# cl-volume-renderer/cl-volume-renderer

Hardware: AMD Instinct MI355X
Metric: msamples_per_sec (higher is better)
Workload: dtype f32

## Files before the change

### cl_volume_renderer_amd/csrc/bounce_device.hpp

```cpp
#pragma once
#include "render_device.hpp"

namespace clvr {

__device__ __forceinline__ VolumePacked make_volume(const RenderArgs &a) {
  return VolumePacked{a.grec, a.stepb, a.volume_lin, a.sdf_lin, a.X, a.Y, a.Z, a.NBX, a.NBY};
}

__device__ __forceinline__ uint32_t udivmod24(uint32_t n, uint32_t d, uint32_t &rem) {
  uint32_t q = (uint32_t)((float)n * __builtin_amdgcn_rcpf((float)d));
  uint32_t qd;
  asm("v_mul_u32_u24 %0, %1, %2" : "=v"(qd) : "v"(q), "v"(d));
  int32_t r = (int32_t)(n - qd);
  if (r < 0) { q -= 1u; r += (int32_t)d; }
  if (r >= (int32_t)d) { q += 1u; r -= (int32_t)d; }
  rem = (uint32_t)r;
  return q;
}

__device__ __forceinline__ unsigned prefix_count(unsigned long long mask) {
  return __builtin_amdgcn_mbcnt_hi((unsigned)(mask >> 32), __builtin_amdgcn_mbcnt_lo((unsigned)mask, 0u));
}
__device__ __forceinline__ unsigned lane_id() { return prefix_count(~0ull); }

enum : int { ST_IDLE = 0, ST_MARCH = 1, ST_CERT = 2, ST_EVENT = 8 };
enum : int { EV_START = 3,
             EV_HIT_COLOR_PENDING = 4,
             EV_CHECK = 5 };
constexpr int kCertNever = 255;

template <int MODE>
__device__ __forceinline__ void finish_item(const RenderArgs &a, int64_t entry, uint32_t hit, uint32_t gx, uint32_t gy,
                                            uint32_t bv_r, uint32_t bv_g, uint32_t bv_b) {
  const uint32_t cr = (bv_r / 2u) & 0xFFFFu, cg = (bv_g / 2u) & 0xFFFFu, cb = (bv_b / 2u) & 0xFFFFu;
  if (MODE == CLWH_ACCUM_VOXEL_CACHE && a.grants == nullptr) {
    cache_add(a.cache, entry, cr, cg, cb, 0u);
  } else {
    const unsigned long long packed = (unsigned long long)cr | ((unsigned long long)cg << 16) |
                                      ((unsigned long long)cb << 32) | (1ull << 48);
    atomicAdd(a.delta + hit, packed);
  }
  if (a.contrib_out) {
    uint32_t *q = a.contrib_out + ((size_t)gy * (size_t)a.launch_w + gx) * 4;
    q[0] = cr; q[1] = cg; q[2] = cb; q[3] = 1u;
  }
}

constexpr int kFixupDwords = 32;

__device__ __forceinline__ bool certify_exit(const RenderArgs &a, f3 p, f3 d, int budget, int &away) {
  const unsigned cx = min((unsigned)(int)p.x >> a.macro_shift, (unsigned)a.MNX - 1u), cy = min((unsigned)(int)p.y >> a.macro_shift, (unsigned)a.MNY - 1u),
                 cz = min((unsigned)(int)p.z >> a.macro_shift, (unsigned)a.MNZ - 1u);
  const unsigned octant = (d.x < 0.0f ? 1u : 0u) | (d.y < 0.0f ? 2u : 0u) | (d.z < 0.0f ? 4u : 0u);
  const int entry = a.macro[(((cz * (unsigned)a.MNY + cy) * (unsigned)a.MNX + cx) << 3) | octant];
  const bool refused = (entry & (int)kCertRefused) != 0;
  const int box_min = refused ? 0 : entry;
  away = refused ? ((entry & 0x7F) - 1) << a.macro_shift : 0;
  const float dmin = fminf(fminf(fabsf(d.x), fabsf(d.y)), fabsf(d.z));
  const float dsum = d.x + d.y + d.z;
  const float T = (float)((budget - 5) * box_min);
  const float fx = d.x < 0.0f ? p.x : (float)a.X - p.x, fy = d.y < 0.0f ? p.y : (float)a.Y - p.y, fz = d.z < 0.0f ? p.z : (float)a.Z - p.z;
  const bool leaves = T * fabsf(d.x) >= fx || T * fabsf(d.y) >= fy || T * fabsf(d.z) >= fz;
  return box_min != 0 && budget > 5 && leaves && dmin >= 0.0009765625f && dsum == dsum;
}
__device__ __forceinline__ bool start_certificate(uint32_t mask, f3 d, float dmin_needed) {
  const unsigned octant = (d.x < 0.0f ? 1u : 0u) | (d.y < 0.0f ? 2u : 0u) | (d.z < 0.0f ? 4u : 0u);
  const float dmin = fminf(fminf(fabsf(d.x), fabsf(d.y)), fabsf(d.z));
  const float dsum = d.x + d.y + d.z;
  return ((mask >> octant) & 1u) != 0u && dmin >= dmin_needed && dsum == dsum;
}
__device__ __forceinline__ f3 hull_direction(unsigned k) {
  static_assert(kHullGrid == 64, "cell centres are odd multiples of 1/64");
  const float u = (float)(2 * (int)(k & 63u) - 63) * 0.015625f, v = (float)(2 * (int)((k >> 6) & 63u) - 63) * 0.015625f;
  const float z = (1.0f - fabsf(u)) - fabsf(v);
  const float x = z >= 0.0f ? u : copysignf(1.0f - fabsf(v), u), y = z >= 0.0f ? v : copysignf(1.0f - fabsf(u), v);
  const float r = __builtin_amdgcn_rsqf((x * x + y * y) + z * z);
  return f3{x * r, y * r, z * r};
}
__device__ __forceinline__ bool certify_exit(const RenderArgs &a, f3 p, f3 d, int budget) {
  int away;
  return certify_exit(a, p, d, budget, away);
}

template <int SMALL>
__device__ __forceinline__ void index_tables_to_lds(VolumePacked &vol, const RenderArgs &a, int threads) {
  extern __shared__ uint32_t lds_parts[];
  if (SMALL == 2) {
    vol.parts = lds_parts;
    vol.parts_y0 = a.X;
    vol.parts_z0 = a.X + a.Y;
    for (int k = (int)threadIdx.x; k < a.X + a.Y + a.Z; k += threads)
      lds_parts[k] = k < a.X ? vol.part_x<1>((unsigned)k) : (k < a.X + a.Y ? vol.part_y<1>((unsigned)(k - a.X)) : vol.part_z<1>((unsigned)(k - a.X - a.Y)));
  }
}
__device__ __forceinline__ unsigned home_queue_of(const RenderArgs &a, unsigned waves_per_block) {
  unsigned home_queue = (unsigned)__builtin_amdgcn_s_getreg((3 << 11) | 20) & 7u;
  if (a.unit_affinity == 1) home_queue = (blockIdx.x * waves_per_block + (threadIdx.x >> 6)) & 7u;
  if (a.unit_affinity == 2) home_queue = 0u;
  return home_queue;
}

#ifdef CLVR_BOUNCE_STATS
constexpr bool kBounceStats = true;
constexpr bool kStartCertVerify = (CLVR_BOUNCE_STATS + 0) != 2;
#else
constexpr bool kBounceStats = false;
constexpr bool kStartCertVerify = false;
#endif
template <bool ON> struct BounceStatsT;
template <> struct BounceStatsT<false> {
  __device__ void step(int) {}
  __device__ void cert_begin(int, int) {}
  __device__ void cert_end(int, int) {}
  __device__ void closing_half(int) {}
  __device__ void event_phase(int) {}
  __device__ void refill(uint32_t) {}
  __device__ void fresh_items(int, int) {}
  __device__ void swap_point() {}
  __device__ void start_cert(bool, bool) {}
  __device__ void hull_cert(bool, bool, bool) {}
  __device__ void hull_more(bool, bool, bool, bool) {}
  __device__ void hull_fired(bool, bool) {}
  __device__ void march_end(uint32_t *, int) {}
  template <bool TWO_RAYS> __device__ void flush(uint32_t *) {}
};
template <> struct BounceStatsT<true> {
  uint32_t step_iters = 0, step_lanes = 0, event_phases = 0, event_lanes = 0, refills = 0, refill_lanes = 0;
  uint32_t ev_kind[4] = {0, 0, 0, 0};
  uint32_t cert_phases = 0, cert_lanes = 0, cert_granted = 0;
  uint32_t step_idle = 0;
  uint32_t swaps = 0;
  uint32_t closing = 0, marching_before = 0;
  __device__ __forceinline__ void step(int st) {
    step_iters += 1; step_lanes += (uint32_t)__popcll(__ballot(st == ST_MARCH));
    step_idle += (uint32_t)__popcll(__ballot(st == ST_IDLE));
  }
  __device__ __forceinline__ void cert_begin(int st, int n_cert) {
    cert_phases += 1; cert_lanes += (uint32_t)n_cert;
    marching_before = (uint32_t)__popcll(__ballot(st == ST_MARCH));
  }
  __device__ __forceinline__ void cert_end(int st, int n_cert) { cert_granted += (uint32_t)(n_cert - (__popcll(__ballot(st == ST_MARCH)) - (int)marching_before)); }
  __device__ __forceinline__ void closing_half(int st) {
    closing = (uint32_t)__popcll(__ballot(st >= ST_EVENT));
    event_lanes += closing;
    ev_kind[1] += (uint32_t)__popcll(__ballot(st == ST_EVENT + EV_EXIT || st == ST_EVENT + EV_CHECK));
    ev_kind[2] += (uint32_t)__popcll(__ballot(st == ST_EVENT + EV_HIT || st == ST_EVENT + EV_HIT_COLOR_PENDING));
    ev_kind[3] += (uint32_t)__popcll(__ballot(st == ST_EVENT + EV_NONE));
  }
  __device__ __forceinline__ void event_phase(int st) {
    if (__ballot(st >= ST_EVENT) != 0ull) { event_phases += 1; event_lanes += (uint32_t)__popcll(__ballot(st >= ST_EVENT)); }
  }
  __device__ __forceinline__ void refill(uint32_t count) { refills += 1; refill_lanes += count; }
  __device__ __forceinline__ void fresh_items(int st, int o) {
    const uint32_t n_fresh = (uint32_t)__popcll(__ballot(st == ST_EVENT + EV_START && o == 1));
    ev_kind[0] += n_fresh; event_lanes += n_fresh;
    if (closing + n_fresh != 0u) event_phases += 1;
  }
  __device__ __forceinline__ void swap_point() { swaps += 1; }
  uint32_t start_tried = 0, start_granted = 0;
  bool start_open = false;
  __device__ __forceinline__ void start_cert(bool tried, bool granted) {
    start_tried += (uint32_t)__popcll(__ballot(tried)); start_granted += (uint32_t)__popcll(__ballot(granted));
    start_open = start_open || granted;
  }
  uint32_t hull_tried = 0, hull_granted = 0, hull_both = 0;
  bool hull_open = false;
  __device__ __forceinline__ void hull_cert(bool tried, bool granted, bool both) {
    hull_tried += (uint32_t)__popcll(__ballot(tried)); hull_granted += (uint32_t)__popcll(__ballot(granted));
    hull_both += (uint32_t)__popcll(__ballot(both));
    hull_open = hull_open || granted;
  }
  uint32_t more_tried[3] = {0, 0, 0}, more_granted[3] = {0, 0, 0};
  int more_open = -1;
  __device__ __forceinline__ void hull_more(bool rebound_tried, bool rebound_granted, bool armed, bool first_leg) {
    more_tried[0] += (uint32_t)__popcll(__ballot(armed && first_leg)); more_tried[2] += (uint32_t)__popcll(__ballot(armed && !first_leg));
    more_tried[1] += (uint32_t)__popcll(__ballot(rebound_tried)); more_granted[1] += (uint32_t)__popcll(__ballot(rebound_granted));
    if (rebound_granted) more_open = 1;
  }
  __device__ __forceinline__ void hull_fired(bool fired, bool first_leg) {
    more_granted[0] += (uint32_t)__popcll(__ballot(fired && first_leg)); more_granted[2] += (uint32_t)__popcll(__ballot(fired && !first_leg));
    if (fired) more_open = first_leg ? 0 : 2;
  }
  __device__ __forceinline__ void march_end(uint32_t *counters, int ev) {
    if (start_open && ev != EV_EXIT) atomicAdd(&counters[CTR_START_WRONG], 1u);
    if (hull_open && ev != EV_EXIT) atomicAdd(&counters[CTR_HULL_WRONG], 1u);
    if (more_open >= 0 && ev != EV_EXIT) atomicAdd(&counters[CTR_HULL_DEFER + 3 * more_open + 2], 1u);
    start_open = false;
    hull_open = false;
    more_open = -1;
  }
  template <bool TWO_RAYS> __device__ __forceinline__ void flush(uint32_t *counters) {
    atomicAdd(&counters[CTR_STEP_ITERS], step_iters); atomicAdd(&counters[CTR_STEP_LANES], step_lanes);
    atomicAdd(&counters[CTR_EVENT_PHASES], event_phases); atomicAdd(&counters[CTR_EVENT_LANES], event_lanes);
    atomicAdd(&counters[CTR_REFILLS], refills); atomicAdd(&counters[CTR_REFILL_LANES], refill_lanes);
    if (TWO_RAYS) { atomicAdd(&counters[CTR_SWAPS], swaps); return; }
    for (int k = 0; k < 4; ++k) atomicAdd(&counters[CTR_EV_KIND + k], ev_kind[k]);
    atomicAdd(&counters[CTR_CERT_PHASES], cert_phases); atomicAdd(&counters[CTR_CERT_LANES], cert_lanes);
    atomicAdd(&counters[CTR_CERT_GRANTED], cert_granted); atomicAdd(&counters[CTR_STEP_IDLE], step_idle);
    atomicAdd(&counters[CTR_START_TRIED], start_tried); atomicAdd(&counters[CTR_START_GRANTED], start_granted);
    atomicAdd(&counters[CTR_HULL_TRIED], hull_tried); atomicAdd(&counters[CTR_HULL_GRANTED], hull_granted); atomicAdd(&counters[CTR_HULL_BOTH], hull_both);
    for (int k = 0; k < 3; ++k) { atomicAdd(&counters[CTR_HULL_DEFER + 3 * k], more_tried[k]); atomicAdd(&counters[CTR_HULL_DEFER + 3 * k + 1], more_granted[k]); }
  }
};
using BounceStats = BounceStatsT<kBounceStats>;

}
```

### cl_volume_renderer_amd/csrc/clwh_context.hip

```cpp
#include <algorithm>
#include <cstdio>
#include <cstdlib>
#include <cstring>
#include <mutex>
#include <new>

#include "clwh_host.hpp"

using namespace clvr;

static thread_local int g_last_hip_error = 0;
void clvr::note_hip_error(hipError_t e) { g_last_hip_error = (int)e; }

static std::atomic<uint64_t> g_content_version{0};
static std::mutex g_cells_mutex;
static std::map<const void *, std::weak_ptr<VersionCell>> g_version_cells;
void clwh_touch(clwh_mem *m) { m->cell->v.store(++g_content_version, std::memory_order_relaxed); }

static std::shared_ptr<VersionCell> version_cell_of(const void *dptr) {
  std::lock_guard<std::mutex> lock(g_cells_mutex);
  auto it = g_version_cells.find(dptr);
  if (it != g_version_cells.end())
    if (auto live = it->second.lock()) return live;
  auto cell = std::make_shared<VersionCell>();
// ... 50 lines not shown
    return rc;
  }
  ctx->classes.cache[source] = j;
  out = j;
  return CLWH_OK;
}

int clvr::ensure_classes(clwh_ctx *ctx, const std::shared_ptr<JitTf> &jit, const clwh_mem *volume, TfDev &tf_out, const uint8_t **cls_out) {
  TfClasses &c = ctx->classes;
  if (c.cls.ptr && c.vol == volume->dptr && c.vol_ver == volume->version() && c.source == jit->source) {
    tf_out = c.tf;
    *cls_out = c.cls.as<uint8_t>();
    return CLWH_OK;
  }
  if (!jit->module) {
    HIP_TRY(hipModuleLoadData(&jit->module, jit->code.data()));
    HIP_TRY(hipModuleGetFunction(&jit->classify, jit->module, "clvr_tf_classify"));
  }
  const size_t voxels = volume->dims[0] * volume->dims[1] * volume->dims[2];
  CLWH_TRY(c.cls.reserve(ctx->stream, voxels));
  constexpr int kColors = CLWH_TF_MAX_RULES;
  CLWH_TRY(c.palette.reserve(ctx->stream, (kColors + 2) * sizeof(unsigned long long)));
  unsigned long long *palette = c.palette.as<unsigned long long>();
  HIP_TRY(hipMemsetAsync(palette, 0xFF, kColors * sizeof(unsigned long long), ctx->stream));
  HIP_TRY(hipMemsetAsync(palette + kColors, 0, 2 * sizeof(unsigned long long), ctx->stream));
  const void *vol = volume->dptr;
  int X = (int)volume->dims[0], Y = (int)volume->dims[1], Z = (int)volume->dims[2], max_colors = kColors;
  unsigned char *cls = c.cls.as<unsigned char>();
  int *error = reinterpret_cast<int *>(palette + kColors);
  int *border = reinterpret_cast<int *>(palette + kColors + 1);
  void *args[] = {&vol, &X, &Y, &Z, &cls, &palette, &max_colors, &error, &border};
  const size_t blocks = std::min<size_t>((voxels + 255u) / 256u, (size_t)1u << 23);
  HIP_TRY(hipModuleLaunchKernel(jit->classify, (unsigned)blocks, 1, 1, 256, 1, 1, 0, ctx->stream, args, nullptr));
  unsigned long long host[kColors + 2];
  HIP_TRY(hipMemcpyAsync(host, palette, sizeof host, hipMemcpyDeviceToHost, ctx->stream));
  HIP_TRY(hipStreamSynchronize(ctx->stream));
  c.vol = nullptr;
  if ((int)(host[kColors] & 0xFFFFFFFFull) != 0) return CLWH_ERR_TF_UNSUPPORTED;
  TfDev t;
  std::memset(&t, 0, sizeof t);
  t.opaque = 1;
  for (int k = 0; k < kColors && host[k] != ~0ull; ++k) {
    t.rules[k].flags = (host[k] >> 32) & 1ull ? TF_WRITES_COLOR : 0u;
    t.rules[k].color = (uint32_t)(host[k] & 0xFFFFFFFFull);
    t.n = k + 1;
  }
  t.border_class = (int32_t)(host[kColors + 1] & 0xFFull);
  c.tf = t;
  c.vol = volume->dptr;
  c.vol_ver = volume->version();
  c.source = jit->source;
  tf_out = t;
  *cls_out = cls;
  return CLWH_OK;
}


Tuning clvr::tuning_from_environment() {
  Tuning t;
  auto clamped = [](const char *e, int lo, int hi) { return std::max(lo, std::min(hi, std::atoi(e))); };
  if (const char *e = std::getenv("CLWH_TUNE_STEP")) t.step_min_lanes = clamped(e, 0, 64);
  if (const char *e = std::getenv("CLWH_TUNE_REFILL")) t.refill_min_lanes = clamped(e, 0, 64);
  if (const char *e = std::getenv("CLWH_TUNE_LITERAL_GRADIENT")) t.literal_gradient = std::atoi(e) != 0;
  if (const char *e = std::getenv("CLWH_TUNE_AFFINITY")) t.unit_affinity = std::atoi(e);
  if (const char *e = std::getenv("CLWH_TUNE_QUEUES")) t.unit_queues = clamped(e, 1, 8);
  if (const char *e = std::getenv("CLWH_TUNE_GROUP")) t.unit_group = std::max(1, std::atoi(e));
  if (const char *e = std::getenv("CLWH_TUNE_CHUNK_BLOCK_LOG2")) t.unit_block_log2 = clamped(e, 0, 8);
  if (const char *e = std::getenv("CLWH_TUNE_BLOCKS")) t.bounce_max_blocks = (uint32_t)std::max(1, std::atoi(e));
  if (const char *e = std::getenv("CLWH_TUNE_MACRO_SHIFT")) t.macro_shift = std::atoi(e);
  if (const char *e = std::getenv("CLWH_TUNE_LONG_LAUNCH")) t.force_long_launch = std::atoi(e) != 0;
  if (const char *e = std::getenv("CLWH_TUNE_BOUNCE_RAYS")) t.bounce_rays = std::atoi(e) == 2 ? 2 : 1;
  if (const char *e = std::getenv("CLWH_TUNE_SDF")) t.sdf_front = std::strcmp(e, "front") == 0;
  if (const char *e = std::getenv("CLWH_TUNE_DIST_LINES")) t.dist_lines = std::strcmp(e, "scan") == 0 ? 1 : std::strcmp(e, "search") == 0 ? 2 : 0;
  if (const char *e = std::getenv("CLWH_TUNE_LABEL_STATS")) t.label_stats = std::strcmp(e, "item") == 0 ? 1 : std::strcmp(e, "direct") == 0 ? 2 : 0;
  if (const char *e = std::getenv("CLWH_TUNE_SLICE_COARSE")) t.slice_coarse = std::atoi(e) != 0;
  if (const char *e = std::getenv("CLWH_TUNE_SDFBIT_WAVES")) t.sdfbit_waves = std::atoi(e) == 16 ? 16 : 8;
  if (const char *e = std::getenv("CLWH_TUNE_SDFBIT_GRID")) t.sdfbit_grid = std::max(1, std::atoi(e));
  if (const char *e = std::getenv("CLWH_TUNE_SDFBIT_REC")) t.sdfbit_rec_lds = std::strcmp(e, "lds") == 0 ? 1 : 0;
  if (const char *e = std::getenv("CLWH_TUNE_CERT")) t.cert_min_step = clamped(e, 0, 127);
  if (const char *e = std::getenv("CLWH_TUNE_CERT_HINT")) t.cert_hint = std::atoi(e) != 0;
  if (const char *e = std::getenv("CLWH_TUNE_START_CERT")) t.start_cert = std::atoi(e) != 0;
  if (const char *e = std::getenv("CLWH_TUNE_HULL_CERT")) t.hull_cert = std::atoi(e) != 0;
  if (const char *e = std::getenv("CLWH_TUNE_HULL_DEFER")) t.hull_defer = std::atoi(e) != 0;
  return t;
}

int clvr::check_device_flags(clwh_ctx *ctx) {
  PassScratch &p = ctx->pass;
  if (!p.fixup_overflow_pending || !p.sticky_flags.ptr) return CLWH_OK;
  uint32_t flag = 0;
  HIP_TRY(hipMemcpyAsync(&flag, p.sticky_flags.ptr, sizeof flag, hipMemcpyDeviceToHost, ctx->stream));
  HIP_TRY(hipStreamSynchronize(ctx->stream));
  p.fixup_overflow_pending = false;
  if (!flag) return CLWH_OK;
  HIP_TRY(hipMemsetAsync(p.sticky_flags.ptr, 0, sizeof(uint32_t), ctx->stream));
  return CLWH_ERR_INTERNAL_OVERFLOW;
}

int clvr::timed_begin(clwh_ctx *ctx, int which, hipEvent_t *end) {
  LaunchTimers &t = ctx->timers;
  if (!t.enabled) return CLWH_OK;
  if (t.used == t.pairs.size()) {
    LaunchTimers::Pair &fresh = t.pairs.emplace_back();
    int rc = fresh.begin.ensure(hipEventDefault);
    if (rc == CLWH_OK) rc = fresh.end.ensure(hipEventDefault);
    if (rc != CLWH_OK) {
      t.pairs.pop_back();
      return rc;
    }
  }
  LaunchTimers::Pair &p = t.pairs[t.used++];
  p.which = which;
  HIP_TRY(hipEventRecord(p.begin.ev, ctx->stream));
  *end = p.end.ev;
  return CLWH_OK;
}

static int order_streams(clwh_ctx *ctx, hipStream_t first, hipStream_t then) {
  HIP_TRY(hipSetDevice(ctx->device));
  CLWH_TRY(ctx->handoff.ensure(hipEventDisableTiming));
  HIP_TRY(hipEventRecord(ctx->handoff.ev, first));
  HIP_TRY(hipStreamWaitEvent(then, ctx->handoff.ev, 0));
  return CLWH_OK;
}

extern "C" {

int clwh_ctx_create_on_stream(int device, void *hip_stream, clwh_ctx **out) {
  if (!out) return CLWH_ERR_INVALID_VALUE;
  *out = nullptr;
  int count = 0;
  hipError_t e = hipGetDeviceCount(&count);
  if (e != hipSuccess || count <= 0) {
    note_hip_error(e);
    return CLWH_ERR_NO_DEVICE;
  }
  if (device < 0 || device >= count) return CLWH_ERR_NO_DEVICE;
  HIP_TRY(hipSetDevice(device));
  clwh_ctx *c = new (std::nothrow) clwh_ctx();
  if (!c) return CLWH_ERR_OUT_OF_MEMORY;
  c->device = device;
  c->stream = (hipStream_t)hip_stream;
  c->own_stream = false;
  c->tune = tuning_from_environment();
  *out = c;
  return CLWH_OK;
}

int clwh_ctx_create(int device, clwh_ctx **out) {
  CLWH_TRY(clwh_ctx_create_on_stream(device, nullptr, out));
  hipStream_t s;
  hipError_t e = hipStreamCreateWithFlags(&s, hipStreamNonBlocking);
  if (e != hipSuccess) {
    note_hip_error(e);
    delete *out;
    *out = nullptr;
    return CLWH_ERR_HIP;
  }
  (*out)->stream = s;
  (*out)->own_stream = true;
  return CLWH_OK;
}

int clwh_ctx_destroy(clwh_ctx *ctx) {
  if (!ctx) return CLWH_ERR_INVALID_VALUE;
  (void)hipSetDevice(ctx->device);
// ... 225 lines not shown
```

### cl_volume_renderer_amd/csrc/clwh_host.hpp

```cpp
#pragma once

#include <atomic>
#include <deque>
#include <map>
#include <memory>
#include <string>
#include <vector>

#include "clwh_internal.hpp"

namespace clvr {

void note_hip_error(hipError_t e);
inline int hip_failed(hipError_t e) {
  note_hip_error(e);
  return e == hipErrorOutOfMemory ? CLWH_ERR_OUT_OF_MEMORY : CLWH_ERR_HIP;
}
#define HIP_TRY(expr)                                   \
  do {                                                  \
    hipError_t _e = (expr);                             \
    if (_e != hipSuccess) return clvr::hip_failed(_e);  \
  } while (0)
#define CLWH_TRY(expr)                \
  do {                                \
// ... 14 lines not shown
  template <class T>
  T *as() const { return static_cast<T *>(ptr); }
  void *release() {
    void *p = ptr;
    ptr = nullptr;
    bytes = 0;
    return p;
  }
  int reserve(hipStream_t stream, size_t need, bool *reallocated = nullptr) {
    if (reallocated) *reallocated = bytes < need;
    if (bytes >= need) return CLWH_OK;
    if (ptr) {
      HIP_TRY(hipStreamSynchronize(stream));
      HIP_TRY(hipFree(ptr));
      (void)release();
    }
    HIP_TRY(hipMalloc(&ptr, need));
    bytes = need;
    return CLWH_OK;
  }
};

struct Event : NoCopy {
  hipEvent_t ev = nullptr;
  ~Event() { if (ev) (void)hipEventDestroy(ev); }
  int ensure(unsigned flags) {
    if (!ev) HIP_TRY(hipEventCreateWithFlags(&ev, flags));
    return CLWH_OK;
  }
};

struct PinnedWord : NoCopy {
  uint32_t *ptr = nullptr;
  ~PinnedWord() { if (ptr) (void)hipHostFree(ptr); }
  int ensure() {
    if (!ptr) HIP_TRY(hipHostMalloc((void **)&ptr, 64, hipHostMallocDefault));
    return CLWH_OK;
  }
};

int tf_jit_compile(const char *user_source, std::vector<char> &code, std::string &log);
struct JitTf {
  std::string source;
  std::vector<char> code;
  hipModule_t module = nullptr;
  hipFunction_t classify = nullptr;
};

struct PackedScene {
  int device = 0;
  DeviceBuffer data;
  const void *vol = nullptr, *sdf = nullptr;
  uint64_t vol_ver = 0, sdf_ver = 0;
  TfDev tf{};
  std::string tf_identity;
  int32_t macro_shift = 0;
  bool start_table = false;
  bool hull_table = false;
  int32_t dims[3] = {0, 0, 0};
  uint64_t generation = 0;
  Event ready;
  bool stale = false;
  ~PackedScene();
};

struct VersionCell {
  std::atomic<uint64_t> v{0};
};


struct Tuning {
  int32_t step_min_lanes = 0;
  int32_t refill_min_lanes = 0;
  int32_t macro_shift = 0;
  int32_t bounce_rays = 1;
  int32_t force_long_launch = 0;
  int32_t literal_gradient = 0;
  int32_t unit_block_log2 = 4;
  int32_t unit_group = 1, unit_affinity = 0, unit_queues = 8;
  int32_t cert_hint = 1;
  int32_t start_cert = 1;
  int32_t hull_cert = 1;
  int32_t hull_defer = 1;
  int32_t cert_min_step = -1;
  uint32_t bounce_max_blocks = 2048;
  int32_t sdfbit_waves = 8;
  int32_t sdfbit_grid = 512;
  int32_t sdfbit_rec_lds = 0;
  int32_t sdf_front = 0;
  int32_t dist_lines = 0;
  int32_t label_stats = 0;
  int32_t slice_coarse = 1;
};
Tuning tuning_from_environment();

struct PrimaryHits {
  struct Key {
    float cam_pos[3], cam_dir[3];
    int32_t frame_w, frame_h, launch_w, launch_h, tile_rank, tile_world;
    int64_t cache_entries;
    int32_t mode, shading;
    uint64_t packed_generation;
    const void *env;
    uint64_t env_version;
    int32_t env_w, env_h;
  } key{};
  bool valid = false;
  DeviceBuffer pix_slot, hits;
  DeviceBuffer hull_codes;
  DeviceBuffer hull_planes;
  uint32_t n_hits = 0;
  bool n_hits_known = false;
  PinnedWord host_n_hits;
  Event n_hits_event;
  bool n_hits_in_flight = false;
  uint32_t last_known_n_hits = 0;
};

struct PassScratch {
  static constexpr size_t kCounters = CTR_QUEUE_STRIDE * 10;
  DeviceBuffer counters;
  DeviceBuffer fixups, delta;
  DeviceBuffer sticky_flags;
  bool fixup_overflow_pending = false;
};

struct VoxelPlan {
  DeviceBuffer plan;
  DeviceBuffer temp;
  bool valid = false;
  uint32_t n = 0;
};

struct TfClasses {
  std::map<std::string, std::shared_ptr<JitTf>> cache;
  DeviceBuffer cls;
  DeviceBuffer palette;
  const void *vol = nullptr;
  uint64_t vol_ver = 0;
  std::string source;
  TfDev tf{};
};

struct SdfScratch {
  DeviceBuffer counters;
  DeviceBuffer flags;
  DeviceBuffer bits;
#ifdef CLVR_SDFBIT_TIMING
  DeviceBuffer timing;
#endif
};

struct TileScratch {
  DeviceBuffer tiles, seeds;
  PinnedWord host;
};

struct GrowScratch {
  DeviceBuffer admissible;
  TileScratch work;
};

struct LabelScratch {
  DeviceBuffer admissible, keys, temp, counters;
  PinnedWord host;
};
// ... 211 lines not shown
```

### cl_volume_renderer_amd/csrc/clwh_internal.hpp

```cpp
#pragma once

#include <hip/hip_runtime.h>
#include <stdint.h>

#include "../../include/clwh.h"

namespace clvr {

struct TfRuleDev {
  int32_t v_lo, v_hi, g_lo, g_hi;
  uint32_t flags;
  uint32_t color;
};
struct TfDev {
  int32_t n;
  int32_t uses_gradient;
  int32_t literal_gradient_taps;
  int32_t opaque;
  int32_t border_class;
  TfRuleDev rules[CLWH_TF_MAX_RULES];
};

enum : uint32_t { TF_USE_GRADIENT = 1u, TF_WRITES_COLOR = 2u, TF_TERMINAL = 4u };

struct HitRec {
  float origin[3];
  float direction[3];
  float normal[3];
  uint32_t color;
  int32_t entry_lo;
  int32_t entry_hi;
  uint32_t xy;
  uint32_t pslot;
  uint32_t start_free;
  uint32_t pad;
};
static_assert(sizeof(HitRec) == 64, "HitRec must be one 64-byte line");

enum : uint32_t { PIX_HIT = 0x80000000u };

constexpr uint32_t kCertMinStep = 2u;
constexpr uint32_t kCertRefused = 0x80u;

enum : uint32_t {
  CTR_HITS = 0, CTR_FIXUPS = 2,
  CTR_STEP_ITERS = 8, CTR_STEP_LANES, CTR_EVENT_PHASES, CTR_EVENT_LANES, CTR_REFILLS, CTR_REFILL_LANES,
  CTR_EV_KIND,
  CTR_CERT_PHASES = CTR_EV_KIND + 4, CTR_CERT_LANES, CTR_CERT_GRANTED,
  CTR_SWAPS, CTR_STEP_IDLE,
  CTR_START_TRIED, CTR_START_GRANTED, CTR_START_WRONG,
  CTR_HULL_TRIED, CTR_HULL_GRANTED, CTR_HULL_BOTH, CTR_HULL_WRONG,
  CTR_STATS_END,
  CTR_QUEUE_STRIDE = 32,
  CTR_HULL_DEFER = CTR_QUEUE_STRIDE * 9, CTR_HULL_DEFER_END = CTR_HULL_DEFER + 9,
};
struct RenderArgs {
  int32_t X, Y, Z;
  const uint2 *grec;
  const uint8_t *stepb;
  const int16_t *volume_lin;
  const int8_t *sdf_lin;
  const uint8_t *macro;
  int32_t MNX, MNY, MNZ, macro_shift;
  int32_t cert_min_step;
  int32_t cert_min_lanes;
  int32_t cert_hint;
  const uint8_t *start_free;
  float start_cert_dmin;
  const float4 *hull;
  uint32_t *hull_codes;
  float hull_delta0;
  uint32_t *hull_planes;
  float hull_defer_delta0;
  int32_t NBX, NBY;
  const uint32_t *env;
  int32_t env_w, env_h;
  uint32_t *cache;
  int64_t cache_entries;
  uint32_t *frame;
  int32_t frame_w, frame_h;
  int32_t launch_w, launch_h;
  int32_t tiles_x, tiles_y, tiles_per_row;
  int32_t tile_rank, tile_world;
  float cam_pos[3];
  float cam_dir[3];
  int32_t mode;
  float4 *accum;
  unsigned long long *delta;
  const uint32_t *grants;
  uint32_t *pix_slot;
  HitRec *hits;
  uint32_t *counters;
  uint32_t *fixups;
  uint32_t fixup_capacity;
  uint32_t *sticky_flags;
  uint32_t n_hits;
  uint32_t n_hits_estimate;
  int32_t n_hits_on_device;
  int32_t shading;
  int64_t *hit_index_out;
  uint32_t *contrib_out;
  uint32_t num_tile_slots;
  int32_t n_seeds;
  int32_t seeds[CLWH_MAX_SEEDS];
  int32_t step_min_lanes;
  int32_t refill_min_lanes;
  int32_t force_long_launch;
  int32_t bounce_rays;
  uint32_t bounce_max_blocks;
  int32_t unit_group;
  int32_t unit_block_log2;
  int32_t unit_queues;
  int32_t unit_affinity;
  TfDev tf;
};

struct RepackArgs {
  const int16_t *volume;
  const int8_t *sdf;
  int32_t X, Y, Z;
  int32_t NBX, NBY, NBZ;
  uint2 *grec;
  uint8_t *stepb;
  uint32_t *brick_min;
  const uint8_t *cls_in;
  TfDev tf;
};

struct SdfArgs {
  const int16_t *volume;
  int32_t X, Y, Z;
  int8_t *ping;
  int8_t *pong;
  int32_t max_iterations;
  int32_t iteration;
  int32_t *counters;
  int32_t *done;
  int32_t *counter_out;
  const uint8_t *cls_in;
  TfDev tf;
};

hipError_t launch_repack(const RepackArgs &a, hipStream_t s);
inline int macro_cell_shift(int X, int Y, int Z, int forced) {
  if (forced >= 3 && forced <= 8) return forced;
  auto cells = [&](int sh) { return (int64_t)((X >> sh) + 1) * ((Y >> sh) + 1) * ((Z >> sh) + 1); };
  int shift = 4;
  if (cells(4) > 40000) {
    shift = 5;
    while (shift < 8 && cells(shift) > 300000) ++shift;
  }
  return shift;
}
hipError_t launch_macro_table(const uint32_t *brick_min, int NBX, int NBY, int NBZ, uint8_t *macro, int X, int Y, int Z, int shift, hipStream_t s);
hipError_t launch_start_table(const uint8_t *stepb, uint8_t *table, uint32_t *regular, int2 *ends, int X, int Y, int Z, int NBX, int NBY, int NBZ, hipStream_t s);
inline int start_cert_cap(int X, int Y, int Z) {
  const int longest = X > Y ? (X > Z ? X : Z) : (Y > Z ? Y : Z);
  return longest / 2 < 127 ? longest / 2 : 127;
}
inline float start_cert_dmin(int X, int Y, int Z) {
  const double longest = (double)(X > Y ? (X > Z ? X : Z) : (Y > Z ? Y : Z));
  const double reach = 1.7320508075688772 * (longest + 1.0), cap = (double)start_cert_cap(X, Y, Z);
  for (int k = 1; k <= 64; ++k) {
    const double dmin = (double)k / 64.0;
    double t = 0.0;
    for (int step = 0; step < 70 - 5 && t <= reach; ++step) {
      const double m = (double)(long long)(t * dmin) - 2.0;
      const double bound = m > cap ? cap : m;
      t += bound < 1.0 ? 1.0 : bound;
    }
    if (t > reach) return (float)dmin;
  }
  return 2.0f;
}
constexpr int kHullGrid = 64;
constexpr int kHullPlanes = kHullGrid * kHullGrid;
constexpr float kHullSlack = 0.0625f;
constexpr int kHullMaxDim = 2048;
inline float hull_cert_delta0(int X, int Y, int Z) {
  const double longest = (double)(X > Y ? (X > Z ? X : Z) : (Y > Z ? Y : Z));
  const double reach = 1.7320508075688772 * (longest + 1.0), cap = (double)start_cert_cap(X, Y, Z);
  for (int k = 1; k <= 64; ++k) {
    const double delta0 = (double)k / 64.0;
    double t = 0.0;
    for (int step = 0; step < 70 - 5 && t <= reach; ++step) {
      const double m = (double)(long long)(t * delta0 / 1.7320508075688772) - 2.0;
      const double bound = m > cap ? cap : m;
      t += bound < 1.0 ? 1.0 : bound;
    }
    if (t > reach) return (float)delta0;
  }
  return 2.0f;
}
constexpr int kHullDeferSteps = 3;
constexpr float kHullDeferDeficit = 1.5f;
constexpr int kHullMarginScale = 16;
inline float hull_defer_delta0(int X, int Y, int Z) {
  const double longest = (double)(X > Y ? (X > Z ? X : Z) : (Y > Z ? Y : Z));
  const double reach = 1.7320508075688772 * (longest + 1.0), cap = (double)start_cert_cap(X, Y, Z);
  for (int k = 1; k <= 64; ++k) {
    const double delta0 = (double)k / 64.0;
    double t = 0.0;
    for (int step = 0; step < 70 - 5 - kHullDeferSteps && t <= reach; ++step) {
      const double m = (double)(long long)(t * delta0 / 1.7320508075688772) - 2.0;
      const double bound = m > cap ? cap : m;
      t += bound < 1.0 ? 1.0 : bound;
    }
    if (t > reach) return (float)delta0;
  }
  return 2.0f;
}
hipError_t launch_hull_table(const int2 *ends, const uint32_t *regular, float4 *hull, int X, int Y, int Z, hipStream_t s);
constexpr uint64_t kStartTableBudget = 2ull << 30;
hipError_t launch_primary(const RenderArgs &a, hipStream_t s);
hipError_t launch_bounce(const RenderArgs &a, hipStream_t s);
inline bool bounce_queues_fit(uint32_t n_hits, int32_t unit_block_log2, int32_t n_seeds) {
  return (uint64_t)(((n_hits + 63u) >> 6) + 8u * (1u << unit_block_log2)) * (uint64_t)n_seeds < (1ull << 24);
}
hipError_t launch_env_fixup(const RenderArgs &a, hipStream_t s);
hipError_t launch_commit(const RenderArgs &a, hipStream_t s);
constexpr int64_t kVoxKeyInvalid = (int64_t)1 << 38;
constexpr int64_t kVoxKeyNone = ((int64_t)1 << 38) + 1;
hipError_t launch_vox_keys(const RenderArgs &a, int64_t *keys, uint32_t *iota, uint32_t n, hipStream_t s);
hipError_t launch_vox_grant(const RenderArgs &a, const int64_t *sorted_keys, const uint32_t *order, uint32_t n, uint32_t *grants, hipStream_t s);
hipError_t launch_commit_voxel(const RenderArgs &a, hipStream_t s);
hipError_t sort_entry_pairs(void *temp, size_t &temp_bytes, const int64_t *keys_in, int64_t *keys_out, const uint32_t *vals_in,
                            uint32_t *vals_out, size_t n, unsigned end_bit, hipStream_t s);
hipError_t launch_resolve(const RenderArgs &a, hipStream_t s);
hipError_t launch_ao(const RenderArgs &a, hipStream_t s);
hipError_t launch_accum_resolve(const RenderArgs &a, const float4 *accum_all, hipStream_t s);
hipError_t launch_accum_resolve_tiles(const RenderArgs &a, const float4 *accum, uint32_t *tiles_out, hipStream_t s);
hipError_t launch_frame_from_tiles(const RenderArgs &a, const uint32_t *tiles_all, hipStream_t s);
struct ProbeShape {
  uint32_t in_words, out_words;
};
ProbeShape probe_shape(int which);
hipError_t launch_device_probe(int which, const uint32_t *in, uint64_t n, uint32_t *out, const uint32_t *aux, const int32_t params[4], hipStream_t s);
struct SdfFrontArgs {
  int8_t *sdf;
  int32_t X, Y, Z;
  int32_t TX, TY, TZ;
  const uint8_t *flags_cur;
  uint8_t *flags_next;
  uint8_t *flags_clear;
  uint8_t *tile_done;
  int32_t iteration;
  int32_t max_iterations;
  int32_t *counters;
};

struct SdfBitArgs {
  int8_t *sdf;
  const uint32_t *ev;
  const uint32_t *r_in;
  uint32_t *r_out;
  uint8_t *state;
  uint8_t *wake;
  int32_t launch;
  int32_t *presence;
  int32_t X, Y, Z, WP;
  int32_t BX, BY, BZ, core_z;
  int32_t r0, steps;
  uint32_t *planes;
  size_t plane_words;
  uint32_t *list;
  uint32_t *list_count;
  uint32_t *list_head;
#ifdef CLVR_SDFBIT_TIMING
  unsigned long long *timing;
#endif
};
void sdfbit_block_grid(int X, int Y, int Z, int waves, int32_t *BX, int32_t *BY, int32_t *BZ, int32_t *core_z);
hipError_t launch_sdfbit_events(const SdfArgs &a, uint32_t *ev, int32_t WP, hipStream_t s);
hipError_t launch_sdfbit_seed(const SdfBitArgs &a, hipStream_t s);
hipError_t launch_sdfbit_expand(const SdfBitArgs &a, const uint32_t *reached, int32_t max_iterations, hipStream_t s);
hipError_t launch_sdfbit_state(const SdfBitArgs &a, hipStream_t s);
hipError_t launch_sdfbit_layers(const SdfBitArgs &a, int waves, unsigned grid_blocks, bool rec_in_lds, hipStream_t s);

inline unsigned row_block(int X) { return X <= 64 ? 64u : (X <= 128 ? 128u : 256u); }
inline dim3 row_grid(int X, int Y, int Z) { return dim3(((unsigned)X + row_block(X) - 1u) / row_block(X), (unsigned)Y, (unsigned)Z); }
hipError_t launch_sdf_base(const SdfArgs &a, hipStream_t s);
hipError_t launch_sdf_base_front(const SdfArgs &a, uint8_t *flags, int32_t TX, int32_t TY, hipStream_t s);
hipError_t launch_sdf_front(const SdfFrontArgs &a, hipStream_t s);
hipError_t launch_sdf_layer(const SdfArgs &a, hipStream_t s);
hipError_t launch_fetch_stats(const int16_t *vol, int X, int Y, int Z, int32_t *stats, hipStream_t s);
hipError_t launch_tf_sort_values(const int16_t *vol, int X, int Y, int Z, uint32_t *frame, int width, int height,
                                 float min_v, float max_v, float min_g, float max_g, hipStream_t s);
hipError_t launch_tf_flush_color_frame(uint32_t *color_frame, int fw, int fh, const int32_t *frame, const int32_t *lookup,
                                       int lookup_len, hipStream_t s);
hipError_t launch_bilateral_filter(const int16_t *src, int X, int Y, int Z, int16_t *dst, const float *weights, hipStream_t s);
hipError_t launch_apply_clip(const int16_t *src, int SX, int SY, int SZ, int16_t *dst, int DX, int DY, int DZ,
                             const uint32_t *start, const uint32_t *len, hipStream_t s);


struct ViewVolume {
// ... 259 lines not shown
```

### cl_volume_renderer_amd/csrc/clwh_render.hip

```cpp
#include <algorithm>
#include <cstdio>
#include <cstring>
#include <mutex>

#include "clwh_host.hpp"

using namespace clvr;


static std::mutex g_scenes_mutex;
static std::vector<std::weak_ptr<PackedScene>> g_packed_scenes;
static std::atomic<uint64_t> g_packed_generation{0};

PackedScene::~PackedScene() {
  (void)hipSetDevice(device);
  (void)hipDeviceSynchronize();
}

struct PackedLayout {
  int X, Y, Z, NBX, NBY, NBZ, mshift, MNX, MNY, MNZ;
  size_t records, n_bricks, off_stepb, off_brick_min, off_macro, off_start, off_hull_ends, off_hull, bytes;
  bool start_table;
  bool hull_table;
};
static bool wants_start_table(const Tuning &t, const TfDev &tf, const clwh_mem *volume) {
  return t.start_cert != 0 && tf.uses_gradient == 0 && tf.border_class == 0 && fits_grid_yz(volume) &&
         (uint64_t)volume->dims[0] * volume->dims[1] * volume->dims[2] <= kStartTableBudget;
}
static bool wants_hull_table(const Tuning &t, const TfDev &tf, const clwh_mem *volume) {
  return t.hull_cert != 0 && wants_start_table(t, tf, volume) && volume->dims[0] <= (size_t)kHullMaxDim && volume->dims[1] <= (size_t)kHullMaxDim &&
         volume->dims[2] <= (size_t)kHullMaxDim;
}
static PackedLayout packed_layout(const clwh_mem *volume, int forced_macro_shift, bool start_table, bool hull_table) {
  PackedLayout L;
  L.X = (int)volume->dims[0]; L.Y = (int)volume->dims[1]; L.Z = (int)volume->dims[2];
  L.NBX = (L.X + 7) / 8; L.NBY = (L.Y + 7) / 8; L.NBZ = (L.Z + 7) / 8;
  L.records = (size_t)L.NBX * L.NBY * L.NBZ * 512u;
  L.n_bricks = (size_t)L.NBX * L.NBY * L.NBZ;
  L.mshift = macro_cell_shift(L.X, L.Y, L.Z, forced_macro_shift);
  const int mcell = 1 << L.mshift;
  L.MNX = (L.X + mcell - 1) >> L.mshift; L.MNY = (L.Y + mcell - 1) >> L.mshift; L.MNZ = (L.Z + mcell - 1) >> L.mshift;
  L.off_stepb = L.records * sizeof(uint2);
  L.off_brick_min = (L.records * (sizeof(uint2) + 1u) + 15u) & ~(size_t)15u;
  L.off_macro = (L.off_brick_min + L.n_bricks * sizeof(uint32_t) + 15u) & ~(size_t)15u;
  L.off_start = (L.off_macro + (size_t)L.MNX * L.MNY * L.MNZ * 8u + 15u) & ~(size_t)15u;
  L.start_table = start_table;
  L.off_hull_ends = (L.off_start + (start_table ? 16u + (size_t)L.X * L.Y * L.Z : 0u) + 15u) & ~(size_t)15u;
  L.hull_table = hull_table;
  L.off_hull = L.off_hull_ends + (hull_table ? (size_t)L.Y * L.Z * sizeof(int2) : 0u);
  L.off_hull = (L.off_hull + 15u) & ~(size_t)15u;
  L.bytes = hull_table ? L.off_hull + (size_t)kHullPlanes * sizeof(float4) : L.off_start + (start_table ? 16u + (size_t)L.X * L.Y * L.Z : 0u);
  return L;
}

static bool packed_matches(const PackedScene &p, int device, const PackedLayout &L, const clwh_mem *volume, const clwh_mem *sdf,
                           const TfDev &tf, const std::string &tf_identity) {
  return !p.stale && p.device == device && p.data.bytes == L.bytes && p.macro_shift == L.mshift && p.start_table == L.start_table && p.hull_table == L.hull_table && p.vol == volume->dptr &&
         p.sdf == sdf->dptr && p.vol_ver == volume->version() && p.sdf_ver == sdf->version() &&
         !std::memcmp(&p.tf, &tf, sizeof tf) && p.tf_identity == tf_identity;
}

static int ensure_packed(clwh_ctx *ctx, const PackedLayout &L, const clwh_mem *volume, const clwh_mem *sdf, const TfDev &tf,
                         const uint8_t *cls_in, const std::string &tf_identity) {
  if (ctx->scene && packed_matches(*ctx->scene, ctx->device, L, volume, sdf, tf, tf_identity)) return CLWH_OK;
  std::shared_ptr<PackedScene> entry;
  {
    std::lock_guard<std::mutex> lock(g_scenes_mutex);
    for (auto it = g_packed_scenes.begin(); it != g_packed_scenes.end();) {
      std::shared_ptr<PackedScene> live = it->lock();
      if (!live) { it = g_packed_scenes.erase(it); continue; }
      if (!entry && packed_matches(*live, ctx->device, L, volume, sdf, tf, tf_identity)) entry = live;
      ++it;
    }
  }
  if (entry) {
    ctx->scene.reset();
    HIP_TRY(hipStreamWaitEvent(ctx->stream, entry->ready.ev, 0));
    ctx->scene = entry;
    return CLWH_OK;
  }
  if (ctx->scene && ctx->scene.use_count() == 1 && ctx->scene->data.bytes == L.bytes) {
    entry = ctx->scene;
  } else {
    ctx->scene.reset();
    entry = std::make_shared<PackedScene>();
    entry->device = ctx->device;
    CLWH_TRY(entry->data.reserve(ctx->stream, L.bytes));
    CLWH_TRY(entry->ready.ensure(hipEventDisableTiming));
  }
  ctx->scene.reset();
  {
    std::lock_guard<std::mutex> lock(g_scenes_mutex);
    entry->stale = true;
  }
  uint8_t *data = entry->data.as<uint8_t>();
  RepackArgs r;
  std::memset(&r, 0, sizeof r);
  r.volume = (const int16_t *)volume->dptr;
  r.sdf = (const int8_t *)sdf->dptr;
  r.X = L.X; r.Y = L.Y; r.Z = L.Z;
  r.NBX = L.NBX; r.NBY = L.NBY; r.NBZ = L.NBZ;
  r.grec = reinterpret_cast<uint2 *>(data);
  r.stepb = data + L.off_stepb;
  r.brick_min = reinterpret_cast<uint32_t *>(data + L.off_brick_min);
  HIP_TRY(hipMemsetAsync(r.brick_min, 0xFF, L.n_bricks * sizeof(uint32_t), ctx->stream));
  r.cls_in = cls_in;
  r.tf = tf;
  CLWH_TRY(timed(ctx, CLWH_TIMER_REPACK, [&] {
    const hipError_t e = launch_repack(r, ctx->stream);
    if (e != hipSuccess) return e;
    return launch_macro_table(r.brick_min, L.NBX, L.NBY, L.NBZ, data + L.off_macro, L.X, L.Y, L.Z, L.mshift, ctx->stream);
  }));
  if (L.start_table)
    CLWH_TRY(timed(ctx, CLWH_TIMER_REPACK, [&] {
      int2 *ends = L.hull_table ? reinterpret_cast<int2 *>(data + L.off_hull_ends) : nullptr;
      const hipError_t e = launch_start_table(r.stepb, data + L.off_start + 16u, reinterpret_cast<uint32_t *>(data + L.off_start), ends, L.X, L.Y, L.Z, L.NBX, L.NBY, L.NBZ, ctx->stream);
      if (e != hipSuccess || !L.hull_table) return e;
      return launch_hull_table(ends, reinterpret_cast<const uint32_t *>(data + L.off_start), reinterpret_cast<float4 *>(data + L.off_hull), L.X, L.Y, L.Z, ctx->stream);
    }));
  HIP_TRY(hipEventRecord(entry->ready.ev, ctx->stream));
  ctx->scene = entry;
  {
    std::lock_guard<std::mutex> lock(g_scenes_mutex);
    entry->vol = volume->dptr;
    entry->sdf = sdf->dptr;
    entry->vol_ver = volume->version();
    entry->sdf_ver = sdf->version();
    entry->tf = tf;
    entry->tf_identity = tf_identity;
    entry->macro_shift = L.mshift;
    entry->start_table = L.start_table;
    entry->hull_table = L.hull_table;
    entry->dims[0] = L.X; entry->dims[1] = L.Y; entry->dims[2] = L.Z;
    entry->generation = ++g_packed_generation;
    entry->stale = false;
    bool listed = false;
    for (auto &w : g_packed_scenes)
      if (w.lock() == entry) listed = true;
    if (!listed) g_packed_scenes.push_back(entry);
  }
  return CLWH_OK;
}


static void describe_frame(RenderArgs &a, int32_t launch_w, int32_t launch_h, int32_t frame_w, int32_t frame_h,
                           int32_t rank, int32_t world, const float cam_pos[3], const float cam_dir[3]) {
  a.launch_w = launch_w;
  a.launch_h = launch_h;
  a.frame_w = frame_w;
  a.frame_h = frame_h;
  a.tiles_x = launch_w / 8;
  a.tiles_y = launch_h / 8;
  a.tile_rank = rank;
  a.tile_world = world;
  a.tiles_per_row = (a.tiles_x + world - 1) / world;
  a.num_tile_slots = (uint32_t)a.tiles_y * (uint32_t)a.tiles_per_row;
  for (int q = 0; q < 3; ++q) {
    a.cam_pos[q] = cam_pos[q];
    a.cam_dir[q] = cam_dir[q];
  }
}

static size_t pixel_slots(const RenderArgs &a) { return (size_t)a.num_tile_slots * 64u; }
static size_t launch_pixels(const RenderArgs &a) { return (size_t)a.launch_w * (size_t)a.launch_h; }
static bool is_planned(const RenderArgs &a) { return a.mode == CLWH_ACCUM_VOXEL_CACHE && a.n_seeds > 1; }

static int validate_desc(const clwh_render_desc *d) {
  if (!is_image(d->volume, 3, 1, CLWH_ELEM_S16) || !is_image(d->sdf, 3, 1, CLWH_ELEM_S8) ||
      !is_image(d->env, 2, 4, CLWH_ELEM_U8))
    return CLWH_ERR_BAD_ARGS;
  if (d->frame && !is_image(d->frame, 2, 4, CLWH_ELEM_U8)) return CLWH_ERR_BAD_ARGS;
  if (!same_dims(d->volume, d->sdf)) return CLWH_ERR_SIZE_MISMATCH;
  if (!launch_size_ok(d->width, d->height)) return CLWH_ERR_BAD_NDRANGE;
  if (d->width > 65535u || d->height > 65535u) return CLWH_ERR_BAD_NDRANGE;
  if (d->env->dims[0] > 32768u || d->env->dims[1] > 32768u) return CLWH_ERR_INVALID_VALUE;
  if (!dims_fit_int32(d->volume)) return CLWH_ERR_INVALID_VALUE;
  const int world = d->tile_world < 1 ? 1 : d->tile_world;
  if (d->tile_rank < 0 || d->tile_rank >= world) return CLWH_ERR_INVALID_VALUE;
  if (d->n_seeds < 0 || d->n_seeds > CLWH_MAX_SEEDS) return CLWH_ERR_INVALID_VALUE;
  if (d->n_seeds > 1 && d->contrib) return CLWH_ERR_BAD_ARGS;
  if (d->shading != CLWH_SHADE_LIGHT && d->shading != CLWH_SHADE_AO) return CLWH_ERR_INVALID_VALUE;
  if (d->shading == CLWH_SHADE_AO && d->accum_mode != CLWH_ACCUM_VOXEL_CACHE) return CLWH_ERR_BAD_ARGS;
  return CLWH_OK;
}

static int describe_launch(const clwh_ctx *ctx, const clwh_render_desc *d, RenderArgs &a) {
  std::memset(&a, 0, sizeof a);
  a.X = (int32_t)d->volume->dims[0];
  a.Y = (int32_t)d->volume->dims[1];
  a.Z = (int32_t)d->volume->dims[2];
  env_into_args(a, d->env);
  const int32_t fw = d->frame ? (int32_t)d->frame->dims[0] : (int32_t)d->width;
  const int32_t fh = d->frame ? (int32_t)d->frame->dims[1] : (int32_t)d->height;
  const int world = d->tile_world < 1 ? 1 : d->tile_world;
  describe_frame(a, (int32_t)d->width, (int32_t)d->height, fw, fh, d->tile_rank, world, d->cam_pos, d->cam_dir);
  a.frame = d->frame ? (uint32_t *)d->frame->dptr : nullptr;
  a.mode = d->accum_mode;
  a.shading = d->shading;
  if (a.mode == CLWH_ACCUM_VOXEL_CACHE) {
    if (!d->buffer_volume || d->buffer_volume->bytes < 8) return CLWH_ERR_BAD_ARGS;
    a.cache = (uint32_t *)d->buffer_volume->dptr;
    a.cache_entries = (int64_t)(d->buffer_volume->bytes / (d->shading == CLWH_SHADE_AO ? 4 : 8));
  } else if (a.mode == CLWH_ACCUM_IMAGE_SPACE) {
    const int64_t need = clwh_accum_len(d->width, d->height, world) * 16;
    if (!d->accum || (int64_t)d->accum->bytes < need) return CLWH_ERR_BAD_ARGS;
    a.accum = (float4 *)d->accum->dptr;
  } else {
    return CLWH_ERR_INVALID_VALUE;
  }
  if (d->hit_index) {
    if (d->hit_index->bytes < launch_pixels(a) * 8) return CLWH_ERR_SIZE_MISMATCH;
    a.hit_index_out = (int64_t *)d->hit_index->dptr;
  }
  if (d->contrib) {
    if (d->contrib->bytes < launch_pixels(a) * 16) return CLWH_ERR_SIZE_MISMATCH;
    a.contrib_out = (uint32_t *)d->contrib->dptr;
  }
  if (d->n_seeds > 0) {
    a.n_seeds = d->n_seeds;
    for (int q = 0; q < d->n_seeds; ++q) a.seeds[q] = d->seeds[q];
  } else {
    a.n_seeds = 1;
    a.seeds[0] = d->seed;
  }
  const Tuning &t = ctx->tune;
  a.step_min_lanes = t.step_min_lanes;
  a.refill_min_lanes = t.refill_min_lanes;
  a.force_long_launch = t.force_long_launch;
  a.bounce_rays = t.bounce_rays;
  a.bounce_max_blocks = t.bounce_max_blocks;
  a.unit_group = t.unit_group;
  a.unit_block_log2 = t.unit_block_log2;
  a.unit_affinity = t.unit_affinity;
  a.unit_queues = t.unit_queues;
  a.cert_hint = t.cert_hint;
  a.start_cert_dmin = start_cert_dmin(a.X, a.Y, a.Z);
  a.hull_delta0 = hull_cert_delta0(a.X, a.Y, a.Z);
  a.hull_defer_delta0 = hull_defer_delta0(a.X, a.Y, a.Z);
  return CLWH_OK;
}

static int bind_scene(clwh_kernel *k, const clwh_render_desc *d, RenderArgs &a) {
  clwh_ctx *ctx = k->ctx;
  const uint8_t *cls_in = nullptr;
  CLWH_TRY(kernel_tf(k, d->volume, a.tf, &cls_in));
  a.tf.literal_gradient_taps = ctx->tune.literal_gradient;
  const PackedLayout L = packed_layout(d->volume, ctx->tune.macro_shift, wants_start_table(ctx->tune, a.tf, d->volume), wants_hull_table(ctx->tune, a.tf, d->volume));
  CLWH_TRY(ensure_packed(ctx, L, d->volume, d->sdf, a.tf, cls_in, k->jit ? k->jit->source : std::string()));
  const uint8_t *packed = ctx->scene->data.as<uint8_t>();
  a.grec = reinterpret_cast<const uint2 *>(packed);
  a.NBX = L.NBX;
  a.NBY = L.NBY;
  a.stepb = packed + L.off_stepb;
  a.volume_lin = (const int16_t *)d->volume->dptr;
  a.sdf_lin = (const int8_t *)d->sdf->dptr;
  a.macro = packed + L.off_macro;
  a.start_free = L.start_table ? packed + L.off_start + 16u : nullptr;
  a.hull = L.hull_table ? reinterpret_cast<const float4 *>(packed + L.off_hull) : nullptr;
  a.macro_shift = L.mshift;
  a.MNX = L.MNX; a.MNY = L.MNY; a.MNZ = L.MNZ;
  bool zero_may_hit = a.tf.border_class != 0;
  for (int q = 0; q < a.tf.n && a.tf.uses_gradient && !a.tf.opaque; ++q)
    if (a.tf.rules[q].v_lo <= 0 && 0 <= a.tf.rules[q].v_hi) zero_may_hit = true;
  const int cert_auto = a.macro_shift < 4 ? 12 >> (4 - a.macro_shift) : std::min(12 << (a.macro_shift - 4), 48);
  a.cert_min_step = zero_may_hit ? 0 : (ctx->tune.cert_min_step >= 0 ? ctx->tune.cert_min_step : cert_auto);
  return CLWH_OK;
}

static int ensure_primary_hits(clwh_ctx *ctx, const clwh_render_desc *d, RenderArgs &a) {
  PrimaryHits &p = ctx->primary;
  PassScratch &s = ctx->pass;
  const size_t slots = pixel_slots(a);
  CLWH_TRY(p.pix_slot.reserve(ctx->stream, slots * sizeof(uint32_t)));
  CLWH_TRY(p.hits.reserve(ctx->stream, slots * sizeof(HitRec)));
  if (a.hull) CLWH_TRY(p.hull_codes.reserve(ctx->stream, slots * sizeof(uint32_t)));
  const bool defer = a.hull && ctx->tune.hull_defer != 0;
  if (defer) CLWH_TRY(p.hull_planes.reserve(ctx->stream, slots * sizeof(uint32_t)));
  CLWH_TRY(s.counters.reserve(ctx->stream, PassScratch::kCounters * sizeof(uint32_t)));
  bool fresh_flags = false;
  CLWH_TRY(s.sticky_flags.reserve(ctx->stream, 64, &fresh_flags));
  if (fresh_flags) HIP_TRY(hipMemsetAsync(s.sticky_flags.ptr, 0, 64, ctx->stream));
  a.sticky_flags = s.sticky_flags.as<uint32_t>();
  a.pix_slot = p.pix_slot.as<uint32_t>();
  a.hits = p.hits.as<HitRec>();
  a.hull_codes = a.hull ? p.hull_codes.as<uint32_t>() : nullptr;
  a.hull_planes = defer ? p.hull_planes.as<uint32_t>() : nullptr;
  a.counters = s.counters.as<uint32_t>();

  PrimaryHits::Key key;
  std::memset(&key, 0, sizeof key);
  for (int q = 0; q < 3; ++q) {
    key.cam_pos[q] = a.cam_pos[q];
    key.cam_dir[q] = a.cam_dir[q];
  }
  key.frame_w = a.frame_w; key.frame_h = a.frame_h;
  key.launch_w = a.launch_w; key.launch_h = a.launch_h;
  key.tile_rank = a.tile_rank; key.tile_world = a.tile_world;
  key.cache_entries = a.cache_entries;
  key.mode = a.mode;
  key.shading = a.shading;
  key.packed_generation = ctx->scene->generation;
  key.env = d->env->dptr;
  key.env_version = d->env->version();
  key.env_w = a.env_w; key.env_h = a.env_h;
  if (p.valid && std::memcmp(&key, &p.key, sizeof key) == 0 && !a.hit_index_out) return CLWH_OK;
  p.valid = false;
  HIP_TRY(hipMemsetAsync(a.counters, 0, PassScratch::kCounters * sizeof(uint32_t), ctx->stream));
  CLWH_TRY(timed(ctx, CLWH_TIMER_PRIMARY, [&] { return launch_primary(a, ctx->stream); }));
  CLWH_TRY(p.host_n_hits.ensure());
  CLWH_TRY(p.n_hits_event.ensure(hipEventDisableTiming));
  HIP_TRY(hipMemcpyAsync(p.host_n_hits.ptr, a.counters + CTR_HITS, sizeof(uint32_t), hipMemcpyDeviceToHost, ctx->stream));
  HIP_TRY(hipEventRecord(p.n_hits_event.ev, ctx->stream));
  p.n_hits_in_flight = true;
  ctx->vox.valid = false;
  p.n_hits_known = false;
  p.key = key;
  p.valid = true;
  return CLWH_OK;
}

static int pick_up_hit_count(clwh_ctx *ctx, RenderArgs &a) {
  PrimaryHits &p = ctx->primary;
  if (p.n_hits_in_flight && !p.n_hits_known) {
    if (hipEventQuery(p.n_hits_event.ev) == hipSuccess) {
      p.n_hits = *p.host_n_hits.ptr;
      p.n_hits_known = true;
      p.n_hits_in_flight = false;
      p.last_known_n_hits = p.n_hits;
    } else {
      (void)hipGetLastError();
    }
  }
  const size_t slots = pixel_slots(a);
  a.n_hits_on_device = !p.n_hits_known;
  a.n_hits = p.n_hits_known ? p.n_hits : (uint32_t)std::min<size_t>(slots, 0xFFFFFFFFu);
  a.n_hits_estimate = a.n_hits;
  if (!p.n_hits_known && p.last_known_n_hits != 0)
    a.n_hits_estimate = (uint32_t)std::min<uint64_t>(a.n_hits, std::max<uint64_t>(2ull * p.last_known_n_hits, slots / 4u));
  if (!bounce_queues_fit(a.n_hits, ctx->tune.unit_block_log2, a.n_seeds)) return CLWH_ERR_INVALID_VALUE;
  return CLWH_OK;
}

static int size_pass_buffers(clwh_ctx *ctx, RenderArgs &a) {
  PassScratch &s = ctx->pass;
  const double rate = std::min(1.0, std::max(1.0 / 64.0, 3.0 * 8.0e-6 * (0.16 * a.env_w + 0.32 * a.env_h)));
  const size_t fix_cap = std::max<size_t>((size_t)((double)a.n_hits_estimate * (double)a.n_seeds * rate), 4096u);
  CLWH_TRY(s.fixups.reserve(ctx->stream, fix_cap * 128u));
  a.fixups = s.fixups.as<uint32_t>();
  a.fixup_capacity = (uint32_t)std::min<size_t>(s.fixups.bytes / 128u, 0x7fffffffu);
  if (a.mode == CLWH_ACCUM_IMAGE_SPACE || is_planned(a)) {
    bool fresh = false;
    CLWH_TRY(s.delta.reserve(ctx->stream, std::max<size_t>(pixel_slots(a), 1) * sizeof(unsigned long long), &fresh));
    a.delta = s.delta.as<unsigned long long>();
    if (fresh) HIP_TRY(hipMemsetAsync(s.delta.ptr, 0, s.delta.bytes, ctx->stream));
  }
  return CLWH_OK;
}

static int plan_voxel_grants(clwh_ctx *ctx, RenderArgs &a) {
  if (!is_planned(a)) return CLWH_OK;
  VoxelPlan &v = ctx->vox;
  constexpr size_t kPerElement = 2 * sizeof(int64_t) + 3 * sizeof(uint32_t);
  bool moved = false;
  CLWH_TRY(v.plan.reserve(ctx->stream, pixel_slots(a) * kPerElement, &moved));
  if (moved) v.valid = false;
  const size_t have = v.plan.bytes / kPerElement;
  int64_t *keys_in = v.plan.as<int64_t>(), *keys = keys_in + have;
  uint32_t *iota = reinterpret_cast<uint32_t *>(keys + have), *order = iota + have, *grants = order + have;
  if (!v.valid) {
    const uint32_t n = a.n_hits;
    HIP_TRY(launch_vox_keys(a, keys_in, iota, n, ctx->stream));
    size_t need = 0;
    HIP_TRY(sort_entry_pairs(nullptr, need, keys_in, keys, iota, order, n, 39u, ctx->stream));
    CLWH_TRY(v.temp.reserve(ctx->stream, std::max<size_t>(need, 16)));
    size_t tb = v.temp.bytes;
    HIP_TRY(sort_entry_pairs(v.temp.ptr, tb, keys_in, keys, iota, order, n, 39u, ctx->stream));
    v.valid = true;
    v.n = n;
  }
  HIP_TRY(launch_vox_grant(a, keys, order, v.n, grants, ctx->stream));
  a.grants = grants;
  return CLWH_OK;
}

#ifdef CLVR_BOUNCE_STATS
static int print_bounce_stats(clwh_ctx *ctx, const RenderArgs &a) {
  uint32_t h[CTR_HULL_DEFER_END];
  HIP_TRY(hipMemcpyAsync(h, a.counters, sizeof h, hipMemcpyDeviceToHost, ctx->stream));
  HIP_TRY(hipStreamSynchronize(ctx->stream));
  auto per = [&](int sum, int n) { return h[n] ? (double)h[sum] / h[n] : 0.0; };
  std::fprintf(stderr, "[bounce stats] items=%llu step_iters=%u avg_march_lanes=%.2f event_phases=%u avg_event_lanes=%.2f "
               "refills=%u avg_refill=%.2f events start/exit/hit/none=%u/%u/%u/%u cert_phases=%u avg_cert_lanes=%.2f cert_granted=%u\n",
               (unsigned long long)h[CTR_HITS] * (unsigned long long)a.n_seeds, h[CTR_STEP_ITERS], per(CTR_STEP_LANES, CTR_STEP_ITERS),
               h[CTR_EVENT_PHASES], per(CTR_EVENT_LANES, CTR_EVENT_PHASES), h[CTR_REFILLS], per(CTR_REFILL_LANES, CTR_REFILLS), h[CTR_EV_KIND],
               h[CTR_EV_KIND + 1], h[CTR_EV_KIND + 2], h[CTR_EV_KIND + 3], h[CTR_CERT_PHASES], per(CTR_CERT_LANES, CTR_CERT_PHASES), h[CTR_CERT_GRANTED]);
  if (h[CTR_SWAPS]) std::fprintf(stderr, "[bounce stats] two rays per lane: %u swap points\n", h[CTR_SWAPS]);
  std::fprintf(stderr, "[bounce stats] per step iteration: avg_idle_lanes=%.2f (lane sum %u)\n", per(CTR_STEP_IDLE, CTR_STEP_ITERS), h[CTR_STEP_IDLE]);
  std::fprintf(stderr, "[bounce stats] lane_steps=%u event_lanes=%u start certificates (%s) tried/granted/wrong=%u/%u/%u dmin=%.6f\n", h[CTR_STEP_LANES],
               h[CTR_EVENT_LANES], (CLVR_BOUNCE_STATS + 0) == 2 ? "taken" : "verified: marched literally", h[CTR_START_TRIED], h[CTR_START_GRANTED],
               h[CTR_START_WRONG], (double)a.start_cert_dmin);
  std::fprintf(stderr, "[bounce stats] hull certificates tried/granted/wrong=%u/%u/%u, of the granted the octant proof grants %u; either proof grants %u first legs; delta0=%.6f\n",
               h[CTR_HULL_TRIED], h[CTR_HULL_GRANTED], h[CTR_HULL_WRONG], h[CTR_HULL_BOTH], h[CTR_START_GRANTED] + h[CTR_HULL_GRANTED] - h[CTR_HULL_BOTH],
               (double)a.hull_delta0);
  const uint32_t *m = h + CTR_HULL_DEFER;
  std::fprintf(stderr, "[bounce stats] hull certificates tried/granted/wrong: first legs deferred=%u/%u/%u rebounds at once=%u/%u/%u rebounds deferred=%u/%u/%u; "
               "J=%d D=%.4g defer_delta0=%.6f; look-ups=%u\n", m[0], m[1], m[2], m[3], m[4], m[5], m[6], m[7], m[8], kHullDeferSteps, (double)kHullDeferDeficit,
               (double)a.hull_defer_delta0, h[CTR_CERT_LANES] - ((CLVR_BOUNCE_STATS + 0) == 2 ? m[1] + m[7] : 0u));
  return CLWH_OK;
}
#endif

static int run_pass(clwh_ctx *ctx, const RenderArgs &a) {
  CLWH_TRY(timed(ctx, CLWH_TIMER_BOUNCE, [&] { return launch_bounce(a, ctx->stream); }));
#ifdef CLVR_BOUNCE_STATS
  CLWH_TRY(print_bounce_stats(ctx, a));
#endif
  CLWH_TRY(timed(ctx, CLWH_TIMER_FIXUP, [&] {
    hipError_t e = launch_env_fixup(a, ctx->stream);
    if (e == hipSuccess) e = launch_commit(a, ctx->stream);
    if (e == hipSuccess && is_planned(a)) e = launch_commit_voxel(a, ctx->stream);
    return e;
  }));
  ctx->pass.fixup_overflow_pending = true;
  return CLWH_OK;
}

extern "C" {

int64_t clwh_cache_len(uint32_t X, uint32_t Y, uint32_t Z) {
  return ((int64_t)X * Z * Y + (int64_t)X * Z + X + 1) * 4;
}

int64_t clwh_accum_len(uint32_t width, uint32_t height, int32_t tile_world) {
  if (tile_world < 1) tile_world = 1;
  const int64_t tiles_x = width / 8, tiles_y = height / 8;
  const int64_t tiles_per_row = (tiles_x + tile_world - 1) / tile_world;
  return tiles_y * tiles_per_row * 64;
}

int clwh_render(clwh_kernel *k, const clwh_render_desc *d) {
  if (!k || !d || k->id != CLWH_K_RENDER || !k->has_tf) return CLWH_ERR_INVALID_VALUE;
  clwh_ctx *ctx = k->ctx;
  RenderArgs a;
  CLWH_TRY(validate_desc(d));
  CLWH_TRY(describe_launch(ctx, d, a));
  HIP_TRY(hipSetDevice(ctx->device));
  CLWH_TRY(bind_scene(k, d, a));
  CLWH_TRY(ensure_primary_hits(ctx, d, a));
  CLWH_TRY(pick_up_hit_count(ctx, a));

  HIP_TRY(hipMemsetAsync(a.counters + CTR_HITS + 1, 0, (PassScratch::kCounters - CTR_HITS - 1) * sizeof(uint32_t), ctx->stream));
  if (a.contrib_out) HIP_TRY(hipMemsetAsync(a.contrib_out, 0, launch_pixels(a) * 16, ctx->stream));

  if (d->resolve_only) {
    if (!a.frame) return CLWH_ERR_BAD_ARGS;
  } else if (d->shading == CLWH_SHADE_AO) {
    CLWH_TRY(timed(ctx, CLWH_TIMER_AO, [&] { return launch_ao(a, ctx->stream); }));
  } else {
    CLWH_TRY(size_pass_buffers(ctx, a));
    CLWH_TRY(plan_voxel_grants(ctx, a));
    CLWH_TRY(run_pass(ctx, a));
  }
  if ((d->write_frame || d->resolve_only) && a.frame)
    CLWH_TRY(timed(ctx, CLWH_TIMER_RESOLVE, [&] { return launch_resolve(a, ctx->stream); }));
  if (d->frame) touch(d->frame);
  return CLWH_OK;
}


int clwh_accum_resolve(clwh_ctx *ctx, clwh_mem *accum_all, int32_t tile_world, uint32_t width, uint32_t height,
                       clwh_mem *frame, clwh_mem *env, const float cam_pos[3], const float cam_dir[3]) {
  if (!ctx || !accum_all || !frame || !env || !cam_pos || !cam_dir || tile_world < 1) return CLWH_ERR_INVALID_VALUE;
  if (!is_image(frame, 2, 4, CLWH_ELEM_U8) || !is_image(env, 2, 4, CLWH_ELEM_U8)) return CLWH_ERR_BAD_ARGS;
  if (!launch_size_ok(width, height)) return CLWH_ERR_BAD_NDRANGE;
  const int64_t need = clwh_accum_len(width, height, tile_world) * 16 * tile_world;
  if ((int64_t)accum_all->bytes < need) return CLWH_ERR_SIZE_MISMATCH;
  RenderArgs a;
  std::memset(&a, 0, sizeof a);
  describe_frame(a, (int32_t)width, (int32_t)height, (int32_t)frame->dims[0], (int32_t)frame->dims[1], 0, tile_world,
                 cam_pos, cam_dir);
  a.frame = (uint32_t *)frame->dptr;
  env_into_args(a, env);
  HIP_TRY(hipSetDevice(ctx->device));
  CLWH_TRY(timed(ctx, CLWH_TIMER_RESOLVE, [&] { return launch_accum_resolve(a, (const float4 *)accum_all->dptr, ctx->stream); }));
  touch(frame);
  return CLWH_OK;
}

int clwh_accum_resolve_tiles(clwh_ctx *ctx, clwh_mem *accum, int32_t tile_rank, int32_t tile_world, uint32_t width, uint32_t height,
                             clwh_mem *tiles_rgba8, clwh_mem *env, const float cam_pos[3], const float cam_dir[3]) {
// ... 98 lines not shown
  info_out[0] = L.NBX; info_out[1] = L.NBY; info_out[2] = L.NBZ; info_out[3] = 0;
  if (!host_out) return CLWH_OK;
  const size_t offset = which == CLWH_SCENE_HIT_RECORDS ? 0u : (which == CLWH_SCENE_STEP_BYTES ? L.off_stepb : L.off_brick_min);
  const size_t bytes = which == CLWH_SCENE_HIT_RECORDS ? L.records * sizeof(uint2) : (which == CLWH_SCENE_STEP_BYTES ? L.records : L.n_bricks * sizeof(uint32_t));
  if (capacity < bytes || ctx->scene->data.bytes != L.bytes) return CLWH_ERR_SIZE_MISMATCH;
  HIP_TRY(hipSetDevice(ctx->device));
  HIP_TRY(hipMemcpyAsync(host_out, ctx->scene->data.as<uint8_t>() + offset, bytes, hipMemcpyDeviceToHost, ctx->stream));
  HIP_TRY(hipStreamSynchronize(ctx->stream));
  return CLWH_OK;
}

int clwh_debug_view_data(clwh_ctx *ctx, int32_t which, void *host_out, uint64_t capacity, int32_t info_out[4]) {
  if (!ctx || !info_out) return CLWH_ERR_INVALID_VALUE;
  if (which != CLWH_VIEW_BRICKS && which != CLWH_VIEW_TABLE && which != CLWH_VIEW_DILATED && which != CLWH_VIEW_COARSE) return CLWH_ERR_INVALID_VALUE;
  const ProjectionData &p = ctx->proj;
  if (!p.valid) return CLWH_ERR_BAD_ARGS;
  const size_t NBX = (p.dims[0] + 7) / 8, NBY = (p.dims[1] + 7) / 8, NBZ = (p.dims[2] + 7) / 8;
  const size_t n_bricks = NBX * NBY * NBZ, n_cells = ((NBX + 3) / 4) * ((NBY + 3) / 4) * ((NBZ + 3) / 4);
  info_out[0] = (int32_t)NBX; info_out[1] = (int32_t)NBY; info_out[2] = (int32_t)NBZ; info_out[3] = (int32_t)n_cells;
  const bool second_level = which == CLWH_VIEW_DILATED || which == CLWH_VIEW_COARSE;
  if (second_level && !p.dilated_valid) return CLWH_ERR_BAD_ARGS;
  if (!host_out) return CLWH_OK;
  const size_t off_table = n_bricks * 512u * sizeof(int16_t);
  const DeviceBuffer &from = second_level ? p.dilated : p.data;
  const size_t offset = which == CLWH_VIEW_TABLE ? off_table : (which == CLWH_VIEW_COARSE ? n_bricks * sizeof(uint32_t) : 0u);
  const size_t bytes = which == CLWH_VIEW_BRICKS ? off_table : (which == CLWH_VIEW_COARSE ? n_cells : n_bricks) * sizeof(uint32_t);
  if (capacity < bytes || from.bytes < offset + bytes) return CLWH_ERR_SIZE_MISMATCH;
  HIP_TRY(hipSetDevice(ctx->device));
  HIP_TRY(hipMemcpyAsync(host_out, from.as<uint8_t>() + offset, bytes, hipMemcpyDeviceToHost, ctx->stream));
  HIP_TRY(hipStreamSynchronize(ctx->stream));
  return CLWH_OK;
}

int clwh_debug_start_table(clwh_ctx *ctx, void *host_out, uint64_t capacity, int32_t info_out[4]) {
  if (!ctx || !info_out) return CLWH_ERR_INVALID_VALUE;
  if (!ctx->scene) return CLWH_ERR_BAD_ARGS;
  const PackedLayout L = scene_layout(ctx);
  info_out[0] = L.X; info_out[1] = L.Y; info_out[2] = L.Z; info_out[3] = L.start_table ? 1 : 0;
  if (!host_out || !L.start_table) return CLWH_OK;
  const size_t bytes = (size_t)L.X * L.Y * L.Z;
  if (capacity < bytes || ctx->scene->data.bytes != L.bytes) return CLWH_ERR_SIZE_MISMATCH;
  HIP_TRY(hipSetDevice(ctx->device));
  HIP_TRY(hipMemcpyAsync(host_out, ctx->scene->data.as<uint8_t>() + L.off_start + 16u, bytes, hipMemcpyDeviceToHost, ctx->stream));
  HIP_TRY(hipStreamSynchronize(ctx->stream));
  return CLWH_OK;
}

int clwh_debug_start_cert_dmin(int32_t X, int32_t Y, int32_t Z, float *dmin_out) {
  if (!dmin_out || X < 1 || Y < 1 || Z < 1) return CLWH_ERR_INVALID_VALUE;
  *dmin_out = start_cert_dmin(X, Y, Z);
  return CLWH_OK;
}

int clwh_debug_hull_table(clwh_ctx *ctx, void *host_out, uint64_t capacity, int32_t info_out[4]) {
  if (!ctx || !info_out) return CLWH_ERR_INVALID_VALUE;
  if (!ctx->scene) return CLWH_ERR_BAD_ARGS;
  const PackedLayout L = scene_layout(ctx);
  info_out[0] = kHullGrid; info_out[1] = kHullPlanes; info_out[2] = 0; info_out[3] = L.hull_table ? 1 : 0;
  if (!host_out || !L.hull_table) return CLWH_OK;
  const size_t bytes = (size_t)kHullPlanes * sizeof(float4);
  if (capacity < bytes || ctx->scene->data.bytes != L.bytes) return CLWH_ERR_SIZE_MISMATCH;
  HIP_TRY(hipSetDevice(ctx->device));
  HIP_TRY(hipMemcpyAsync(host_out, ctx->scene->data.as<uint8_t>() + L.off_hull, bytes, hipMemcpyDeviceToHost, ctx->stream));
  HIP_TRY(hipStreamSynchronize(ctx->stream));
  return CLWH_OK;
}

int clwh_debug_hull_cert_bound(int32_t X, int32_t Y, int32_t Z, float out[2]) {
  if (!out || X < 1 || Y < 1 || Z < 1) return CLWH_ERR_INVALID_VALUE;
  out[0] = hull_cert_delta0(X, Y, Z);
  out[1] = kHullSlack;
  return CLWH_OK;
}

int clwh_debug_hull_defer_bound(int32_t X, int32_t Y, int32_t Z, float out[4]) {
  if (!out || X < 1 || Y < 1 || Z < 1) return CLWH_ERR_INVALID_VALUE;
  out[0] = hull_defer_delta0(X, Y, Z);
  out[1] = (float)kHullDeferSteps;
  out[2] = kHullDeferDeficit;
  out[3] = (float)kHullMarginScale;
  return CLWH_OK;
}

int clwh_debug_hull_planes(clwh_ctx *ctx, void *host_out, uint64_t capacity, uint32_t *n_hits_out) {
  if (!ctx || !n_hits_out) return CLWH_ERR_INVALID_VALUE;
  PrimaryHits &p = ctx->primary;
  if (!p.valid || !p.hits.ptr || !ctx->pass.counters.ptr) return CLWH_ERR_BAD_ARGS;
  HIP_TRY(hipSetDevice(ctx->device));
  HIP_TRY(hipMemcpyAsync(n_hits_out, ctx->pass.counters.as<uint32_t>() + CTR_HITS, sizeof(uint32_t), hipMemcpyDeviceToHost, ctx->stream));
  HIP_TRY(hipStreamSynchronize(ctx->stream));
  if (!host_out) return CLWH_OK;
  const bool built = ctx->scene && ctx->scene->hull_table && ctx->tune.hull_defer != 0 && p.hull_planes.ptr;
  const size_t bytes = (size_t)*n_hits_out * sizeof(uint32_t);
  if (capacity < bytes || (built && p.hull_planes.bytes < bytes)) return CLWH_ERR_SIZE_MISMATCH;
  if (!built) { std::memset(host_out, 0, bytes); return CLWH_OK;}
  HIP_TRY(hipMemcpyAsync(host_out, p.hull_planes.ptr, bytes, hipMemcpyDeviceToHost, ctx->stream));
  HIP_TRY(hipStreamSynchronize(ctx->stream));
  return CLWH_OK;
}

int clwh_debug_hull_codes(clwh_ctx *ctx, void *host_out, uint64_t capacity, uint32_t *n_hits_out) {
  if (!ctx || !n_hits_out) return CLWH_ERR_INVALID_VALUE;
  PrimaryHits &p = ctx->primary;
  if (!p.valid || !p.hits.ptr || !ctx->pass.counters.ptr) return CLWH_ERR_BAD_ARGS;
  HIP_TRY(hipSetDevice(ctx->device));
  HIP_TRY(hipMemcpyAsync(n_hits_out, ctx->pass.counters.as<uint32_t>() + CTR_HITS, sizeof(uint32_t), hipMemcpyDeviceToHost, ctx->stream));
  HIP_TRY(hipStreamSynchronize(ctx->stream));
  if (!host_out) return CLWH_OK;
  const bool built = ctx->scene && ctx->scene->hull_table && p.hull_codes.ptr;
  const size_t bytes = (size_t)*n_hits_out * sizeof(uint32_t);
  if (capacity < bytes || (built && p.hull_codes.bytes < bytes)) return CLWH_ERR_SIZE_MISMATCH;
  if (!built) { std::memset(host_out, 0, bytes); return CLWH_OK; }
  HIP_TRY(hipMemcpyAsync(host_out, p.hull_codes.ptr, bytes, hipMemcpyDeviceToHost, ctx->stream));
  HIP_TRY(hipStreamSynchronize(ctx->stream));
  return CLWH_OK;
}

int clwh_debug_hit_records(clwh_ctx *ctx, void *host_out, uint64_t capacity, uint32_t *n_hits_out) {
  if (!ctx || !n_hits_out) return CLWH_ERR_INVALID_VALUE;
  PrimaryHits &p = ctx->primary;
  if (!p.valid || !p.hits.ptr || !ctx->pass.counters.ptr) return CLWH_ERR_BAD_ARGS;
  HIP_TRY(hipSetDevice(ctx->device));
  HIP_TRY(hipMemcpyAsync(n_hits_out, ctx->pass.counters.as<uint32_t>() + CTR_HITS, sizeof(uint32_t), hipMemcpyDeviceToHost, ctx->stream));
  HIP_TRY(hipStreamSynchronize(ctx->stream));
  if (!host_out) return CLWH_OK;
  const size_t bytes = (size_t)*n_hits_out * sizeof(HitRec);
  if (capacity < bytes || p.hits.bytes < bytes) return CLWH_ERR_SIZE_MISMATCH;
  HIP_TRY(hipMemcpyAsync(host_out, p.hits.ptr, bytes, hipMemcpyDeviceToHost, ctx->stream));
  HIP_TRY(hipStreamSynchronize(ctx->stream));
  return CLWH_OK;
}

}
```

### cl_volume_renderer_amd/csrc/probe_kernels.hip

```cpp
#include "render_device.hpp"

namespace clvr {

__host__ __device__ __forceinline__ ProbeShape probe_shape_of(int which) {
  switch (which) {
    case CLWH_PROBE_ARITH: return {6u, 12u};
    case CLWH_PROBE_HASH: return {1u, 1u};
    case CLWH_PROBE_HEMISPHERE: return {7u, 6u};
    case CLWH_PROBE_RAY: return {10u, 3u};
    case CLWH_PROBE_CUT: return {6u, 4u};
    case CLWH_PROBE_ENV_EXACT: return {3u, 1u};
    case CLWH_PROBE_ENV_FAST: return {3u, 2u};
    case CLWH_PROBE_ENV_APPROX: return {3u, 2u};
    case CLWH_PROBE_TONE: return {4u, 1u};
    case CLWH_PROBE_TAPS: return {3u, 3u};
    default: return {0u, 0u};
  }
}

struct ProbeParams {
  int32_t v[4];
};

__device__ __forceinline__ f3 f3_at(const uint32_t *r) {
  return f3{__uint_as_float(r[0]), __uint_as_float(r[1]), __uint_as_float(r[2])};
}
__device__ __forceinline__ void put_f3(uint32_t *o, f3 v) {
  o[0] = __float_as_uint(v.x);
  o[1] = __float_as_uint(v.y);
  o[2] = __float_as_uint(v.z);
}

__global__ __launch_bounds__(256) void k_debug_device_probe(int which, const uint32_t *__restrict__ in, uint64_t n,
                                                            uint32_t *__restrict__ out, const uint32_t *__restrict__ aux,
                                                            ProbeParams params) {
  const uint64_t i = (uint64_t)blockIdx.x * 256u + threadIdx.x;
  if (i >= n) return;
  const ProbeShape shape = probe_shape_of(which);
  const uint32_t *r = in + i * shape.in_words;
  uint32_t *o = out + i * shape.out_words;
  switch (which) {
    case CLWH_PROBE_ARITH: {
      const f3 a = f3_at(r), b = f3_at(r + 3);
      o[0] = __float_as_uint(a.x / b.x);
      o[1] = __float_as_uint(sqrtf(a.x));
      o[2] = __float_as_uint(dot3(a, b));
      o[3] = __float_as_uint(length3(a));
      put_f3(o + 4, normalize3(a));
      put_f3(o + 7, cross3(a, b));
      o[10] = __float_as_uint(cl_min(a.x, b.x));
      o[11] = __float_as_uint(cl_max(a.x, b.x));
      break;
    }
    case CLWH_PROBE_HASH: o[0] = hash_u32(r[0]); break;
    case CLWH_PROBE_HEMISPHERE: {
      const f3 normal = f3_at(r + 2);
      const int seed = (int)r[5];
      put_f3(o, hemisphere_reflective(r[0], r[1], normal, seed, __uint_as_float(r[6])));
      put_f3(o + 3, hemisphere_direction(r[0], r[1], normal, seed));
      break;
    }
    case CLWH_PROBE_RAY: {
      const Ray ray = generate_ray(f3_at(r), f3_at(r + 3), (int)r[6], (int)r[7], (int)r[8], (int)r[9]);
      put_f3(o, ray.direction);
      break;
    }
    case CLWH_PROBE_CUT: {
      f3 point;
      const bool hit = cut_box((float)params.v[0], (float)params.v[1], (float)params.v[2], Ray{f3_at(r), f3_at(r + 3)}, point);
      o[0] = hit ? 1u : 0u;
      put_f3(o + 1, point);
      break;
    }
    case CLWH_PROBE_ENV_EXACT: o[0] = sample_environment_map(aux, params.v[0], params.v[1], f3_at(r)); break;
    case CLWH_PROBE_ENV_FAST: {
      uint32_t texel = 0xFFFFFFFFu;
      const bool decided = sample_environment_map_fast(aux, params.v[0], params.v[1], f3_at(r), texel);
      o[0] = decided ? 1u : 0u;
      o[1] = decided ? texel : 0xFFFFFFFFu;
      break;
    }
    case CLWH_PROBE_ENV_APPROX:
      o[0] = __float_as_uint(atan2_approx(__uint_as_float(r[0]), __uint_as_float(r[1])));
      o[1] = __float_as_uint(asin_approx(__uint_as_float(r[2])));
      break;
    case CLWH_PROBE_TONE: o[0] = tone_map_rgba8(r[0], r[1], r[2], r[3]); break;
    case CLWH_PROBE_TAPS: {
      const f3 p = f3_at(r);
      const int64_t e = cache_entry_of(params.v[0], params.v[1], p);
      o[0] = taps_are_voxel_neighbours(p) ? 1u : 0u;
      o[1] = (uint32_t)((uint64_t)e & 0xFFFFFFFFu);
      o[2] = (uint32_t)((uint64_t)e >> 32);
      break;
    }
    default: break;
  }
}

ProbeShape probe_shape(int which) { return probe_shape_of(which); }

hipError_t launch_device_probe(int which, const uint32_t *in, uint64_t n, uint32_t *out, const uint32_t *aux, const int32_t params[4], hipStream_t s) {
  ProbeParams p;
  for (int k = 0; k < 4; ++k) p.v[k] = params[k];
  hipLaunchKernelGGL(k_debug_device_probe, dim3((unsigned)((n + 255u) / 256u)), dim3(256), 0, s, which, in, n, out, aux, p);
  return hipGetLastError();
}

}
```

### cl_volume_renderer_amd/csrc/render_kernels.hip

```cpp
#include <algorithm>

#include "bounce_two_rays.hpp"

namespace clvr {

#ifndef CLVR_CERT_PHASE_MIN_LANES
#define CLVR_CERT_PHASE_MIN_LANES 16
#endif
constexpr int kCertPhaseMinLanes = CLVR_CERT_PHASE_MIN_LANES;
#ifndef CLVR_BOUNCE_WAVES_PER_SIMD
#define CLVR_BOUNCE_WAVES_PER_SIMD 7
#endif
#ifndef CLVR_BOUNCE_THREADS
#define CLVR_BOUNCE_THREADS 256
#endif
constexpr int kBounceThreads = CLVR_BOUNCE_THREADS;

template <bool USE_GRAD, int MODE, bool SMALL_VOLUME>
__global__ __launch_bounds__(kBounceThreads, CLVR_BOUNCE_WAVES_PER_SIMD) void k_bounce(const RenderArgs a) {
  constexpr int SMALL = SMALL_VOLUME ? 2 : 0;
  VolumePacked vol = make_volume(a);
  index_tables_to_lds<SMALL>(vol, a, kBounceThreads);
  __shared__ float div255[256];
  if (threadIdx.x < 256u) div255[threadIdx.x] = (float)threadIdx.x / 255.0f;
  __syncthreads();
  const uint32_t n_hits = a.n_hits_on_device ? a.counters[CTR_HITS] : a.n_hits;
  const uint32_t n_chunks = (n_hits + 63u) >> 6;
  const unsigned lane = lane_id();
  const unsigned home_queue = home_queue_of(a, (unsigned)(kBounceThreads / 64));
  unsigned queue_dry = 0u;
  enum : int { C_START_X, C_START_Y, C_START_Z,
               C_NORMAL_X, C_NORMAL_Y, C_NORMAL_Z,
               C_ENTRY_LO,
               C_ENTRY_HI,
               C_PIXEL, C_HIT, C_SEED,
               C_FIX,
               C_BV_R, C_BV_G, C_BV_B, C_FIELDS };
  __shared__ uint32_t cold[C_FIELDS][kBounceThreads];
#define COLD(f) cold[f][threadIdx.x]
#define COLD_ENTRY_HI() ((uint32_t)((int32_t)(COLD(C_ENTRY_HI) << (32 - entry_hi_bits)) >> (32 - entry_hi_bits)))
  Ray ray{{0, 0, 0}, {0, 0, 0}};
  float atten = 0.0f, r_energy = 0.0f, g_energy = 0.0f, b_energy = 0.0f;
  uint32_t color = 0u;
  int o = 0, i = 0;
  int st = ST_IDLE;
  int sd = 0;
  uint32_t march = 0u;
  constexpr uint32_t kOneStep = 1u << 24, kCertReady = 1u << 23, kArmed = 1u << 31;
  const bool cert_hint = a.cert_hint != 0;
  const int cert_min_lanes = a.cert_min_lanes;
  const int cert_at = a.cert_min_step != 0 ? a.cert_min_step : kCertNever;
  const bool start_cert = !USE_GRAD && a.cert_min_step != 0;
  const bool hull_cert = start_cert && a.hull_codes != nullptr;
  const bool hull_defer = hull_cert && a.hull_planes != nullptr;
  const int entry_hi_bits = hull_defer ? 3 : 8;
  const uint32_t *hull_words = hull_defer ? a.hull_planes : a.hull_codes;
  bool exhausted = false;
  BounceStats stats;

  for (;;) {
    if (__ballot(st == ST_MARCH) != 0ull) {
      do {
        stats.step(st);
        if (st == ST_MARCH) {
          ray.origin = ray.origin + ray.direction * fmaxf((float)sd, 0.5f);
          march += (uint32_t)sd - kOneStep;
          if (!USE_GRAD) {
            const bool has_voxel = __float_as_uint(ray.origin.x) < __float_as_uint((float)a.X) &&
                                   __float_as_uint(ray.origin.y) < __float_as_uint((float)a.Y) &&
                                   __float_as_uint(ray.origin.z) < __float_as_uint((float)a.Z);
            if (has_voxel) {
              const unsigned q = vol.template step_marched<SMALL>(ray.origin.x, ray.origin.y, ray.origin.z);
              sd = (int)(q & 0x7Fu);
              if (q & 0x80u) st = ST_EVENT + EV_HIT_COLOR_PENDING;
              else if ((march & ~kArmed) < kOneStep) st = ST_EVENT + EV_NONE;
              else if (((march & kArmed) | (uint32_t)sd) >= (uint32_t)cert_at && (march & kCertReady)) st = ST_CERT;
            } else {
              st = ST_EVENT + EV_CHECK;
            }
          } else if (exited_volume(vol, ray.origin)) {
            st = ST_EVENT + EV_EXIT;
          } else {
            int next_sd;
            bool pending = false;
            const bool is_hit = classify_step<USE_GRAD, SMALL, true>(vol, a.tf, ray.origin, color, next_sd, &pending);
            if (is_hit) {
              st = ST_EVENT + (pending ? EV_HIT_COLOR_PENDING : EV_HIT);
            } else if (march < kOneStep) {
              st = ST_EVENT + EV_NONE;
            } else {
              sd = next_sd;
              if (sd >= cert_at && (march & kCertReady)) st = ST_CERT;
            }
          }
        }
        const int n_cert = __popcll(__ballot(st == ST_CERT));
        if (n_cert != 0 && (n_cert >= cert_min_lanes || __popcll(__ballot(st == ST_MARCH)) < a.step_min_lanes)) {
          stats.cert_begin(st, n_cert);
          const bool fired = !USE_GRAD && st == ST_CERT && (march & kArmed) != 0u && (march & ~kArmed) >= (uint32_t)(70 - kHullDeferSteps) * kOneStep;
          stats.hull_fired(fired, i == 8);
          if (st == ST_CERT) {
            if (!USE_GRAD) march &= ~kArmed;
            int away;
            if (fired && !kStartCertVerify) {
              st = ST_EVENT + EV_EXIT;
            } else if (certify_exit(a, ray.origin, ray.direction, (int)(march >> 24), away)) {
              st = ST_EVENT + EV_EXIT;
            } else {
              march = (march & ~(kOneStep - 1u)) | (kCertReady - (uint32_t)(cert_hint ? away : 0));
              st = ST_MARCH;
            }
          }
          stats.cert_end(st, n_cert);
        }
      } while (__popcll(__ballot(st == ST_MARCH)) >= a.step_min_lanes);
    }

    stats.closing_half(st);
    if (st >= ST_EVENT) {
      int ev = st - ST_EVENT;
      if (ev == EV_CHECK) {
        for (;;) {
          if (exited_volume(vol, ray.origin)) { ev = EV_EXIT; break; }
          int next_sd;
          bool pending = false;
          if (classify_step<USE_GRAD, SMALL, true>(vol, a.tf, ray.origin, color, next_sd, &pending)) {
            ev = pending ? EV_HIT_COLOR_PENDING : EV_HIT;
            break;
          }
          if ((march & ~kArmed) < kOneStep) { ev = EV_NONE; break; }
          ray.origin = ray.origin + ray.direction * fmaxf((float)next_sd, 0.5f);
          march -= kOneStep;
        }
      }
      stats.march_end(a.counters, ev);
      bool ended = false;

      if (ev == EV_EXIT) {
        const float factor = i == 8 ? 8.0f / 8.0f : (i == 9 ? 8.0f / 9.0f : (i == 10 ? 8.0f / 10.0f : 8.0f / (float)i));
        const float p_r = atten * r_energy, p_g = atten * g_energy, p_b = atten * b_energy;
        uint32_t light = 0u;
        const uint32_t fix_word = COLD(C_FIX);
        int fix = (int)(fix_word >> 2) - 2, npend = (int)(fix_word & 3u);
        bool certain = (fix == -1) && sample_environment_map_fast(a.env, a.env_w, a.env_h, ray.direction, light);
        if (certain) {
          COLD(C_BV_R) = f2u((float)COLD(C_BV_R) + p_r * (float)(light & 255u) * factor / 1.0f);
          COLD(C_BV_G) = f2u((float)COLD(C_BV_G) + p_g * (float)((light >> 8) & 255u) * factor / 1.0f);
          COLD(C_BV_B) = f2u((float)COLD(C_BV_B) + p_b * (float)((light >> 16) & 255u) * factor / 1.0f);
        } else {
          if (fix == -1) {
            const uint32_t slot = atomicAdd(&a.counters[CTR_FIXUPS], 1u);
            if (slot < a.fixup_capacity) {
              fix = (int)slot;
              uint32_t *rec = a.fixups + (size_t)slot * kFixupDwords;
              rec[0] = COLD(C_HIT);
              rec[1] = COLD(C_ENTRY_LO);
              rec[2] = COLD_ENTRY_HI();
              rec[3] = COLD(C_PIXEL);
              rec[4] = COLD(C_BV_R); rec[5] = COLD(C_BV_G); rec[6] = COLD(C_BV_B);
            } else {
              a.sticky_flags[0] = 1u;
              fix = -2;
            }
          }
          if (fix >= 0) {
            uint32_t *e = a.fixups + (size_t)fix * kFixupDwords + 8 + 7 * npend;
            e[0] = __float_as_uint(p_r); e[1] = __float_as_uint(p_g); e[2] = __float_as_uint(p_b);
            e[3] = __float_as_uint(factor);
            e[4] = __float_as_uint(ray.direction.x); e[5] = __float_as_uint(ray.direction.y);
            e[6] = __float_as_uint(ray.direction.z);
            npend += 1;
          }
          COLD(C_FIX) = ((uint32_t)(fix + 2) << 2) | (uint32_t)npend;
        }
        o += 1;
        ev = EV_START;
        ended = true;
      } else if (ev == EV_HIT || ev == EV_HIT_COLOR_PENDING) {
        i += 1;
        if (i > 10) {
          o += 1;
          ended = true;
        }
      } else if (ev == EV_NONE) {
        i += 1;
        if (i > 10) {
          o += 1;
          ev = EV_START;
// ... 18 lines not shown
    if (!exhausted && n_idle >= (uint32_t)a.refill_min_lanes) {
      const uint32_t NQ = (uint32_t)a.unit_queues, S = (uint32_t)a.n_seeds, G = (uint32_t)a.unit_group;
      const uint32_t KB = (uint32_t)a.unit_block_log2, n_blocks = (n_chunks + (1u << KB) - 1u) >> KB;
      uint32_t base = 0u, count = 0u, q_sel = 0u;
      if (lane == 0u) {
        for (uint32_t tries = 0; tries < NQ && count == 0u; ++tries) {
          const uint32_t q = (home_queue + tries) % NQ;
          const uint32_t blocks_q = (n_blocks + NQ - 1u - q) / NQ;
          const uint32_t chunks_q = blocks_q << KB;
          if (chunks_q == 0u || ((queue_dry >> q) & 1u)) continue;
          const uint32_t total = chunks_q * S * 64u;
          const uint32_t p = atomicAdd(&a.counters[CTR_QUEUE_STRIDE * (q + 1u)], n_idle);
          if (p + n_idle >= total) queue_dry |= 1u << q;
          if (p < total) {
            base = p;
            count = min(n_idle, total - p);
            q_sel = q;
          }
        }
      }
      base = __shfl(base, 0);
      count = __shfl(count, 0);
      q_sel = __shfl(q_sel, 0);
      stats.refill(count);
      if (count == 0u) {
        exhausted = true;
      } else if (st == ST_IDLE) {
        const uint32_t rank = (uint32_t)__popcll(idle_mask & ((1ull << lane) - 1ull));
        if (rank < count) {
          const uint32_t item = base + rank, p = item >> 6;
          const uint32_t chunks_q = ((n_blocks + NQ - 1u - q_sel) / NQ) << KB;
          uint32_t r, c_in;
          const uint32_t g = udivmod24(p, G * S, r);
          const uint32_t in_group = min(G, chunks_q - g * G);
          const uint32_t s = udivmod24(r, in_group, c_in), ch = g * G + c_in;
          const uint32_t chunk = ((q_sel + NQ * (ch >> KB)) << KB) + (ch & ((1u << KB) - 1u));
          const uint32_t h = chunk * 64u + (item & 63u);
          if (h < n_hits) {
            const uint4 *src = reinterpret_cast<const uint4 *>(&a.hits[h]);
            const uint4 q0 = src[0], q1 = src[1], q2 = src[2], q3 = src[3];
            const f3 hit_origin = f3{__uint_as_float(q0.x), __uint_as_float(q0.y), __uint_as_float(q0.z)};
            const f3 hit_direction = f3{__uint_as_float(q0.w), __uint_as_float(q1.x), __uint_as_float(q1.y)};
            const f3 start = hit_origin + hit_direction;
            color = q2.y;
            const int64_t entry = (int64_t)(((uint64_t)q2.w << 32) | (uint64_t)q2.z);
            bool granted = true;
            if (MODE == CLWH_ACCUM_VOXEL_CACHE)
              granted = a.grants ? s < a.grants[h] : (entry >= 0 && cache_take_token(a.cache, entry, 256u));
            if (granted) {
              COLD(C_START_X) = __float_as_uint(start.x); COLD(C_START_Y) = __float_as_uint(start.y); COLD(C_START_Z) = __float_as_uint(start.z);
              COLD(C_NORMAL_X) = q1.z; COLD(C_NORMAL_Y) = q1.w; COLD(C_NORMAL_Z) = q2.x;
              COLD(C_ENTRY_LO) = q2.z;
              const uint32_t plane = hull_cert ? hull_words[h] : 0u;
              COLD(C_ENTRY_HI) = (q2.w & ((1u << entry_hi_bits) - 1u)) | ((plane & 0x1FFFu) << entry_hi_bits) | (plane & (hull_defer ? 0x00FF0000u : 0u)) | (q3.z << 24);
              COLD(C_PIXEL) = q3.x;
              COLD(C_HIT) = h;
              COLD(C_SEED) = (uint32_t)a.seeds[s];
              COLD(C_FIX) = (uint32_t)(-1 + 2) << 2;
              COLD(C_BV_R) = 0u; COLD(C_BV_G) = 0u; COLD(C_BV_B) = 0u;
              r_energy = div255[color & 255u];
              g_energy = div255[(color >> 8) & 255u];
              b_energy = div255[(color >> 16) & 255u];
              o = 1;
              st = ST_EVENT + EV_START;
            } else if (a.contrib_out) {
              uint32_t *q = a.contrib_out + ((size_t)(q3.x >> 16) * (size_t)a.launch_w + (q3.x & 0xFFFFu)) * 4;
              q[0] = 0u; q[1] = 0u; q[2] = 0u; q[3] = 0u;
            }
          }
        }
      }
    }
    stats.fresh_items(st, o);
    if (__ballot(st != ST_IDLE) == 0ull) {
      if (exhausted && lane == 0u) stats.flush<false>(a.counters);
      if (exhausted) break;
      continue;
    }

    bool sc_tried = false, sc_granted = false;
    bool hc_tried = false, hc_granted = false;
    bool rb_tried = false, rb_granted = false;
    uint32_t armed_path = 0u;
    if (st >= ST_EVENT) {
      const int ev = st - ST_EVENT;
      bool start_path = (ev == EV_START);
      bool bounce = false, from_hit = false;
      f3 bn{0, 0, 0}, bstart{0, 0, 0};
      int bseed = 0;

      if (ev == EV_HIT || ev == EV_HIT_COLOR_PENDING) {
        bn = -normalize3(hit_gradient_and_color<SMALL>(vol, a.tf, ray.origin, ev == EV_HIT_COLOR_PENDING, color));
        bstart = ray.origin + ray.direction;
        bseed = o + i - 1;
        bounce = true;
        from_hit = true;
        if (i > 10) {
          r_energy *= div255[color & 255u];
          g_energy *= div255[(color >> 8) & 255u];
          b_energy *= div255[(color >> 16) & 255u];
          bounce = false;
          start_path = true;
        }
      }

      if (start_path) {
        bn = f3{__uint_as_float(COLD(C_NORMAL_X)), __uint_as_float(COLD(C_NORMAL_Y)), __uint_as_float(COLD(C_NORMAL_Z))};
        bstart = f3{__uint_as_float(COLD(C_START_X)), __uint_as_float(COLD(C_START_Y)), __uint_as_float(COLD(C_START_Z))};
        bseed = o;
        bounce = true;
        from_hit = false;
      }

      if (bounce) {
        const float roughness = div255[color >> 24];
        const uint32_t pixel = COLD(C_PIXEL);
        Ray nr;
        nr.direction = hemisphere_reflective(pixel & 0xFFFFu, pixel >> 16, bn, (int)COLD(C_SEED) + bseed, roughness);
        nr.origin = bstart + bn * 2.0f;
        const float d = fabsf(dot3(nr.direction, bn));
        if (from_hit) {
          atten *= d;
          r_energy *= div255[color & 255u];
          g_energy *= div255[(color >> 8) & 255u];
          b_energy *= div255[(color >> 16) & 255u];
        } else {
          atten = d;
          i = 8;
          if (start_cert) {
            sc_tried = true;
            const uint32_t word = COLD(C_ENTRY_HI);
            sc_granted = start_certificate(word >> 24, nr.direction, a.start_cert_dmin);
          }
        }
        if (hull_cert && (hull_defer || !from_hit)) {
          const uint32_t word = COLD(C_ENTRY_HI);
          const uint32_t code = (word >> entry_hi_bits) & 0x1FFFu;
          const f3 n = hull_direction(code - 1u);
          const float dn = dot3(nr.direction, n);
          const f3 dir = nr.direction;
          const bool dir_ok = fminf(fminf(fabsf(dir.x), fabsf(dir.y)), fabsf(dir.z)) >= 0.0009765625f && (dir.x + dir.y) + dir.z == (dir.x + dir.y) + dir.z;
          float m = hull_defer ? (float)((int32_t)(word << 8) >> 24) * (1.0f / (float)kHullMarginScale) : 0.0f;
          if (from_hit) {
            const f3 p = f3{__uint_as_float(COLD(C_START_X)), __uint_as_float(COLD(C_START_Y)), __uint_as_float(COLD(C_START_Z))} +
                         f3{__uint_as_float(COLD(C_NORMAL_X)), __uint_as_float(COLD(C_NORMAL_Y)), __uint_as_float(COLD(C_NORMAL_Z))} * 2.0f;
            m = m + dot3(n, f3{nr.origin.x - p.x, nr.origin.y - p.y, nr.origin.z - p.z});
          }
          const bool tried = code != 0u, granted = tried && dir_ok && m >= 0.0f && dn >= a.hull_delta0;
          if (from_hit) { rb_tried = tried; rb_granted = granted; }
          else { hc_tried = tried && m >= 0.0f; hc_granted = granted; }
          if (tried && dir_ok && !sc_granted && m < 0.0f && m >= -kHullDeferDeficit && dn >= a.hull_defer_delta0)
            armed_path = (uint32_t)ceilf(-m * __builtin_amdgcn_rcpf(dn) * (1.0f + 0x1p-19f));
        }
        ray = nr;
      }

      if ((sc_granted || hc_granted || rb_granted) && !kStartCertVerify) {
        st = ST_EVENT + EV_EXIT;
      } else {
        sd = (int)(vol.template step_i<SMALL>(f2i(ray.origin.x), f2i(ray.origin.y), f2i(ray.origin.z)) & 0x7Fu);
        march = 70u * kOneStep + kCertReady;
        if (armed_path != 0u) march = kArmed + 70u * kOneStep + kCertReady - armed_path;
        st = ST_MARCH;
      }
    }
    stats.start_cert(sc_tried, sc_granted);
    stats.hull_cert(hc_tried, hc_granted, hc_granted && sc_granted);
    stats.hull_more(rb_tried, rb_granted, armed_path != 0u && st == ST_MARCH, i == 8);
  }
#undef COLD_ENTRY_HI
#undef COLD
}

hipError_t launch_bounce(const RenderArgs &a_in, hipStream_t s) {
  RenderArgs a = a_in;
  const uint64_t total = (uint64_t)a.n_hits * (uint64_t)a.n_seeds;
  if (total == 0) return hipSuccess;
  const uint64_t waves_needed = (total + 63u) / 64u;
  constexpr unsigned wpb = (unsigned)kBounceThreads / 64u;
  const unsigned blocks = (unsigned)std::min<uint64_t>((waves_needed + wpb - 1u) / wpb, ((uint64_t)a.bounce_max_blocks * 4u + wpb - 1u) / wpb);
  const dim3 grid(blocks), block(kBounceThreads);
  const uint64_t waves_likely = ((uint64_t)a.n_hits_estimate * (uint64_t)a.n_seeds + 63u) / 64u;
  const bool long_launch = a.force_long_launch || waves_likely >= 6u * (uint64_t)blocks * wpb;
  if (a.step_min_lanes <= 0) a.step_min_lanes = long_launch ? 16 : 1;
  if (a.refill_min_lanes <= 0) a.refill_min_lanes = long_launch ? 16 : 64;
  a.cert_min_lanes = kCertPhaseMinLanes;
  if (!long_launch) a.cert_min_step = 0;
  if (!bounce_queues_fit(a.n_hits, a.unit_block_log2, a.n_seeds)) return hipErrorInvalidValue;
  const bool g = a.tf.uses_gradient != 0;
  const bool small = (uint64_t)a.NBX * (uint64_t)a.NBY * (uint64_t)((a.Z + 7) / 8) < (1ull << 23) &&
                     a.X + a.Y + a.Z <= VolumePacked::kPartsMaxEntries;
  const size_t lds_parts_bytes = small ? (size_t)(a.X + a.Y + a.Z) * sizeof(uint32_t) : 0u;
  const bool two_rays = a.bounce_rays == 2 && long_launch && a.n_hits < (1u << 26) && kBounceThreads == 256;
  if (two_rays) a.fixup_capacity = std::min<uint32_t>(a.fixup_capacity, (1u << 27) - 4u);
#define CLVR_LAUNCH_BOUNCE(G, M)                                                                    \
  do {                                                                                              \
    if (two_rays) {                                                                                 \
      if (small) hipLaunchKernelGGL((k_bounce2<G, M, true>), grid, block, lds_parts_bytes, s, a);  \
      else hipLaunchKernelGGL((k_bounce2<G, M, false>), grid, block, 0, s, a);                     \
    } else if (small) hipLaunchKernelGGL((k_bounce<G, M, true>), grid, block, lds_parts_bytes, s, a); \
    else hipLaunchKernelGGL((k_bounce<G, M, false>), grid, block, 0, s, a);                        \
  } while (0)
  if (a.mode == CLWH_ACCUM_VOXEL_CACHE) {
    if (g) CLVR_LAUNCH_BOUNCE(true, CLWH_ACCUM_VOXEL_CACHE);
    else CLVR_LAUNCH_BOUNCE(false, CLWH_ACCUM_VOXEL_CACHE);
  } else {
    if (g) CLVR_LAUNCH_BOUNCE(true, CLWH_ACCUM_IMAGE_SPACE);
    else CLVR_LAUNCH_BOUNCE(false, CLWH_ACCUM_IMAGE_SPACE);
  }
#undef CLVR_LAUNCH_BOUNCE
  return hipGetLastError();
}

}
```

### cl_volume_renderer_amd/csrc/scene_kernels.hip

```cpp
#include "bounce_device.hpp"

namespace clvr {

#ifndef CLVR_REPACK_X
#define CLVR_REPACK_X 64
#endif
constexpr int kRepackX = CLVR_REPACK_X;
constexpr int kRepackPitch = kRepackX + 16;
constexpr int kRepackX0 = 8;
__global__ __launch_bounds__(256) void k_repack(const RepackArgs a) {
  __shared__ __attribute__((aligned(16))) int16_t s_val[10][10][kRepackPitch];
  __shared__ __attribute__((aligned(16))) int8_t s_sdf[8][8][kRepackX];
  const int x0 = (int)blockIdx.x * kRepackX, y0 = (int)blockIdx.y * 8, z0 = (int)blockIdx.z * 8;
  const unsigned tid = threadIdx.x;
  if ((a.X & 15) == 0 && x0 + kRepackX <= a.X && ((reinterpret_cast<uintptr_t>(a.volume) | reinterpret_cast<uintptr_t>(a.sdf)) & 15u) == 0u) {
    constexpr unsigned kChunks = kRepackX / 8;
    for (unsigned i = tid; i < 10u * 10u * kChunks; i += 256u) {
      const unsigned row = i / kChunks, c = i % kChunks;
      const int ry = (int)(row % 10u), rz = (int)(row / 10u);
      const int y = y0 - 1 + ry, z = z0 - 1 + rz;
      uint4 v = uint4{0u, 0u, 0u, 0u};
      int16_t left = 0, right = 0;
      if ((unsigned)y < (unsigned)a.Y && (unsigned)z < (unsigned)a.Z) {
        const int16_t *src = a.volume + ((size_t)z * (size_t)a.Y + (size_t)y) * (size_t)a.X + (size_t)x0;
// ... 209 lines not shown
      for (int c = 0; c < 8; ++c)
        m = min(m, at(min(max(x + ((c & 1) ? 1 : -1), 0), X - 1), min(max(y + ((c & 2) ? 1 : -1), 0), Y - 1), min(max(z + ((c & 4) ? 1 : -1), 0), Z - 1)) & 0x7Fu);
      ok = ok && s >= min(cap, m + 1u);
    } else {
      bool touches = false;
      for (int dz = -1; dz <= 1; ++dz)
        for (int dy = -1; dy <= 1; ++dy)
          for (int dx = -1; dx <= 1; ++dx)
            touches = touches || (at(min(max(x + dx, 0), X - 1), min(max(y + dy, 0), Y - 1), min(max(z + dz, 0), Z - 1)) & 0x80u) != 0u;
      ok = ok && touches && (s == 1u || (q & 0x80u) != 0u);
    }
  }
  if (!ok) *regular = 0u;
}
__global__ __launch_bounds__(256) void k_start_rows(const uint8_t *__restrict__ stepb, uint8_t *__restrict__ table, int2 *__restrict__ ends, int X, int Y, int Z, int NBX, int NBY) {
  const int lane = (int)(threadIdx.x & 63u), y = (int)blockIdx.x * 4 + (int)(threadIdx.x >> 6);
  if (y >= Y) return;
  for (int k = 0; k < 4; ++k) {
    const int z = (int)blockIdx.y * 4 + k;
    if (z >= Z) break;
    int first = X, last = -1;
    for (int x0 = 0; x0 < X; x0 += 64) {
      const int x = x0 + lane;
      const unsigned long long ev = __ballot(x < X && (stepb[VolumePacked::record_index(min(x, X - 1), y, z, NBX, NBY)] & 0x80u) != 0u);
      if (ev != 0ull) {
        if (first == X) first = x0 + __ffsll((long long)ev) - 1;
        last = x0 + 63 - __clzll((long long)ev);
      }
    }
    uint8_t *row = table + ((size_t)z * (size_t)Y + (size_t)y) * (size_t)X;
    for (int x = lane; x < X; x += 64) row[x] = (uint8_t)((x > last ? 0x55u : 0u) | (x < first ? 0xAAu : 0u));
    if (ends != nullptr && lane == 0) ends[(size_t)z * (size_t)Y + (size_t)y] = make_int2(first, last);
  }
}
__global__ __launch_bounds__(256) void k_start_scan(uint8_t *__restrict__ table, int X, int Y, int Z, int axis, const uint32_t *regular) {
  const int x = (int)(blockIdx.x * blockDim.x + threadIdx.x), other = (int)blockIdx.y;
  if (x >= X) return;
  const int len = axis == 1 ? Y : Z;
  const size_t stride = axis == 1 ? (size_t)X : (size_t)X * (size_t)Y;
  uint8_t *line = table + (axis == 1 ? (size_t)other * (size_t)Y * (size_t)X : (size_t)other * (size_t)X) + (size_t)x;
  const unsigned up = axis == 1 ? 0x33u : 0x0Fu;
  const unsigned keep = (regular == nullptr || *regular != 0u) ? 0xFFu : 0u;
  unsigned run = 0xFFu;
  for (int i = len - 1; i >= 0; --i) {
    const unsigned v = line[(size_t)i * stride];
    run &= v;
    line[(size_t)i * stride] = (uint8_t)((v & ~up) | (run & up));
  }
  run = 0xFFu;
  for (int i = 0; i < len; ++i) {
    const unsigned v = line[(size_t)i * stride];
    run &= v;
    line[(size_t)i * stride] = (uint8_t)(((v & up) | (run & ~up)) & keep);
  }
}
hipError_t launch_start_table(const uint8_t *stepb, uint8_t *table, uint32_t *regular, int2 *ends, int X, int Y, int Z, int NBX, int NBY, int NBZ, hipStream_t s) {
  hipError_t e = hipMemsetAsync(regular, 1, sizeof(uint32_t), s);
  if (e != hipSuccess) return e;
  hipLaunchKernelGGL(k_start_regular, dim3((unsigned)(NBX * NBY * NBZ)), dim3(256), 0, s, stepb, X, Y, Z, NBX, NBY, (unsigned)start_cert_cap(X, Y, Z), regular);
  hipLaunchKernelGGL(k_start_rows, dim3(((unsigned)Y + 3u) / 4u, ((unsigned)Z + 3u) / 4u), dim3(256), 0, s, stepb, table, ends, X, Y, Z, NBX, NBY);
  hipLaunchKernelGGL(k_start_scan, dim3(((unsigned)X + 255u) / 256u, (unsigned)Z), dim3(256), 0, s, table, X, Y, Z, 1, (const uint32_t *)nullptr);
  hipLaunchKernelGGL(k_start_scan, dim3(((unsigned)X + 255u) / 256u, (unsigned)Y), dim3(256), 0, s, table, X, Y, Z, 2, (const uint32_t *)regular);
  return hipGetLastError();
}

constexpr int kHullRows = 512;
__device__ __forceinline__ uint32_t ordered_bits(float v) {
  const uint32_t b = __float_as_uint(v);
  return (b & 0x80000000u) ? ~b : (b | 0x80000000u);
}
__global__ __launch_bounds__(256) void k_hull_support(const int2 *__restrict__ ends, int Y, int n_rows, uint32_t *__restrict__ best_out) {
  const unsigned k = blockIdx.x * 256u + threadIdx.x;
  const f3 n = hull_direction(k);
  const int r0 = (int)blockIdx.y * kHullRows, r1 = min(r0 + kHullRows, n_rows);
  float best = -INFINITY;
  for (int r = r0; r < r1; ++r) {
    const int2 e = ends[r];
    if (e.y < 0) continue;
    const float yz = n.y * (float)(r % Y) + n.z * (float)(r / Y);
    best = fmaxf(best, yz + fmaxf(n.x * (float)e.x, n.x * (float)e.y));
  }
  if (best > -INFINITY) atomicMax(&best_out[4u * k + 3u], ordered_bits(best));
}
__global__ __launch_bounds__(256) void k_hull_finish(const uint32_t *__restrict__ regular, float4 *__restrict__ hull) {
  const unsigned k = blockIdx.x * 256u + threadIdx.x;
  const f3 n = hull_direction(k);
  const uint32_t o = reinterpret_cast<const uint32_t *>(hull)[4u * k + 3u];
  const uint32_t b = (o & 0x80000000u) ? (o & 0x7FFFFFFFu) : ~o;
  float h = INFINITY;
  if (o != 0u && *regular != 0u) h = (__uint_as_float(b) + ((fmaxf(n.x, 0.0f) + fmaxf(n.y, 0.0f)) + fmaxf(n.z, 0.0f))) + kHullSlack;
  hull[k] = make_float4(n.x, n.y, n.z, h);
}
hipError_t launch_hull_table(const int2 *ends, const uint32_t *regular, float4 *hull, int X, int Y, int Z, hipStream_t s) {
  (void)X;
  const hipError_t e = hipMemsetAsync(hull, 0, (size_t)kHullPlanes * sizeof(float4), s);
  if (e != hipSuccess) return e;
  const int n_rows = Y * Z;
  hipLaunchKernelGGL(k_hull_support, dim3((unsigned)kHullPlanes / 256u, ((unsigned)n_rows + (unsigned)kHullRows - 1u) / (unsigned)kHullRows), dim3(256), 0, s, ends, Y, n_rows,
                     reinterpret_cast<uint32_t *>(hull));
  hipLaunchKernelGGL(k_hull_finish, dim3((unsigned)kHullPlanes / 256u), dim3(256), 0, s, regular, hull);
  return hipGetLastError();
}

}
```

### cl_volume_renderer_amd/ffi.py

```python
from __future__ import annotations

import ctypes as C
import os

import numpy as np

_HERE = os.path.dirname(os.path.abspath(__file__))
LIB_PATH = os.environ.get("CLWH_LIBRARY") or os.path.join(_HERE, "libclwhip.so")

OK = 0
ELEM_S8, ELEM_S16, ELEM_S32, ELEM_U8, ELEM_U16, ELEM_U32, ELEM_F32 = range(7)
ARG_MEM, ARG_I32, ARG_U32, ARG_F32, ARG_I64, ARG_U64, ARG_F64 = range(7)
ACCUM_VOXEL_CACHE, ACCUM_IMAGE_SPACE = 0, 1
DERIVED_SCENE, DERIVED_CAMERA, DERIVED_PROJECTION = 1, 2, 4
PROJ_MAX, PROJ_MIN, PROJ_MEAN = 0, 1, 2
PROJ_DENSE = 1
COMP_DENSE, COMP_SHADE = 1, 2
ISO_DENSE, ISO_BELOW = 1, 2
SLICE_MAX, SLICE_MIN, SLICE_MEAN = 0, 1, 2
SLICE_DENSE = 1
MESH_DENSE, MESH_BELOW = 1, 2
GROW_26, GROW_FROM_MASK, GROW_DENSE = 1, 2, 4
GROW_MAX_SEEDS = 65536
LABEL_26, LABEL_FROM_MASK = 1, 2
DIST_NONE = 0xFFFFFFFF
DIST_TO_CLEAR = 1
GEO_26, GEO_FROM_LABELS, GEO_DENSE = 1, 2, 4
GEO_CAP_MAX = 0xFFFF0000
MORPH_DILATE, MORPH_ERODE, MORPH_OPEN, MORPH_CLOSE = 0, 1, 2, 3
MASK_AND, MASK_OR, MASK_XOR, MASK_ANDNOT, MASK_NOT = 0, 1, 2, 3, 4
MASK_INVERT = 1
REGION_MASK, REGION_LABELS = 0, 1
OVERLAY_FILL, OVERLAY_OUTLINE, OVERLAY_DENSE = 1, 2, 4
SHADE_LIGHT, SHADE_AO = 0, 1
(PROBE_ARITH, PROBE_HASH, PROBE_HEMISPHERE, PROBE_RAY, PROBE_CUT, PROBE_ENV_EXACT, PROBE_ENV_FAST, PROBE_ENV_APPROX, PROBE_TONE,
 PROBE_TAPS) = range(10)
PROBE_WORDS = ((6, 12), (1, 1), (7, 6), (10, 3), (6, 4), (3, 1), (3, 2), (3, 2), (4, 1), (3, 3))
SCENE_HIT_RECORDS, SCENE_STEP_BYTES, SCENE_BRICK_MIN = range(3)
VIEW_BRICKS, VIEW_TABLE, VIEW_DILATED, VIEW_COARSE = range(4)
TIMERS = ("bounce", "primary", "fixup", "resolve", "repack", "ao")
MAX_SEEDS = 64
TF_MAX_RULES = 16

_ELEM_OF_DTYPE = {
    np.dtype(np.int8): ELEM_S8, np.dtype(np.int16): ELEM_S16, np.dtype(np.int32): ELEM_S32,
    np.dtype(np.uint8): ELEM_U8, np.dtype(np.uint16): ELEM_U16, np.dtype(np.uint32): ELEM_U32,
    np.dtype(np.float32): ELEM_F32,
}


class ClwhError(RuntimeError):
    def __init__(self, status, where):
        self.status = status
        name = lib().clwh_strerror(status).decode()
        super().__init__("%s failed: %s (hip error %d)" % (where, name, lib().clwh_last_hip_error()))


class _ArgValue(C.Union):
    _fields_ = [("mem", C.c_void_p), ("i32", C.c_int32), ("u32", C.c_uint32), ("f32", C.c_float),
                ("i64", C.c_int64), ("u64", C.c_uint64), ("f64", C.c_double)]


class Arg(C.Structure):
    _fields_ = [("kind", C.c_int32), ("reserved", C.c_int32), ("v", _ArgValue)]


class TfRule(C.Structure):
    _fields_ = [("v_lo", C.c_int32), ("v_hi", C.c_int32), ("g_lo", C.c_int32), ("g_hi", C.c_int32),
                ("use_gradient", C.c_int32), ("writes_color", C.c_int32), ("terminal", C.c_int32),
                ("color", C.c_int32 * 4)]


class Tf(C.Structure):
    _fields_ = [("n", C.c_int32), ("rules", TfRule * TF_MAX_RULES)]

    def as_tuples(self):
        return [(r.v_lo, r.v_hi, r.g_lo, r.g_hi, r.use_gradient, r.writes_color, r.terminal, tuple(r.color))
                for r in list(self.rules)[: self.n]]


class RenderDesc(C.Structure):
    _fields_ = [
        ("frame", C.c_void_p), ("volume", C.c_void_p), ("sdf", C.c_void_p), ("env", C.c_void_p),
        ("buffer_volume", C.c_void_p),
        ("cam_pos", C.c_float * 3), ("cam_dir", C.c_float * 3), ("seed", C.c_int32),
        ("width", C.c_uint32), ("height", C.c_uint32),
        ("accum_mode", C.c_int32), ("accum", C.c_void_p),
        ("tile_rank", C.c_int32), ("tile_world", C.c_int32),
        ("write_frame", C.c_int32),
        ("hit_index", C.c_void_p), ("contrib", C.c_void_p),
        ("n_seeds", C.c_int32), ("seeds", C.c_int32 * 64),
        ("shading", C.c_int32), ("resolve_only", C.c_int32),
    ]


class ProjectionDesc(C.Structure):
    _fields_ = [
        ("frame", C.c_void_p), ("volume", C.c_void_p),
        ("cam_pos", C.c_float * 3), ("cam_dir", C.c_float * 3),
        ("width", C.c_uint32), ("height", C.c_uint32),
        ("mode", C.c_int32), ("flags", C.c_int32),
        ("step", C.c_float), ("t_near", C.c_float), ("t_far", C.c_float),
        ("window_center", C.c_float), ("window_width", C.c_float),
        ("values", C.c_void_p), ("t_extreme", C.c_void_p),
    ]


class CompositeDesc(C.Structure):
    _fields_ = [
        ("frame", C.c_void_p), ("volume", C.c_void_p),
        ("cam_pos", C.c_float * 3), ("cam_dir", C.c_float * 3),
        ("width", C.c_uint32), ("height", C.c_uint32),
        ("flags", C.c_int32),
        ("step", C.c_float), ("t_near", C.c_float), ("t_far", C.c_float),
        ("lut", C.c_void_p), ("lut_first", C.c_int32), ("lut_len", C.c_int32),
        ("alpha_stop", C.c_float), ("ambient", C.c_float),
        ("rgba", C.c_void_p), ("t_first", C.c_void_p), ("t_stop", C.c_void_p),
    ]


# ... 198 lines not shown
    ]


class OverlayCameraDesc(C.Structure):
    _fields_ = [
        ("frame", C.c_void_p), ("region", OverlayRegion), ("paint", OverlayPaint),
        ("cam_pos", C.c_float * 3), ("cam_dir", C.c_float * 3),
        ("width", C.c_uint32), ("height", C.c_uint32),
        ("step", C.c_float), ("t_near", C.c_float), ("t_far", C.c_float), ("reserved", C.c_int32),
    ]


_SIZE3 = C.POINTER(C.c_size_t)
_PROTOTYPES = [
    ("clwh_ctx_create", C.c_int, [C.c_int, C.POINTER(C.c_void_p)]),
    ("clwh_ctx_create_on_stream", C.c_int, [C.c_int, C.c_void_p, C.POINTER(C.c_void_p)]),
    ("clwh_ctx_destroy", C.c_int, [C.c_void_p]),
    ("clwh_ctx_finish", C.c_int, [C.c_void_p]),
    ("clwh_ctx_stream", C.c_void_p, [C.c_void_p]),
    ("clwh_ctx_device", C.c_int, [C.c_void_p]),
    ("clwh_mem_create", C.c_int, [C.c_void_p, C.c_size_t, C.c_int, C.POINTER(C.c_void_p)]),
    ("clwh_mem_wrap", C.c_int, [C.c_void_p, C.c_void_p, C.c_size_t, C.POINTER(C.c_void_p)]),
    ("clwh_image_create", C.c_int, [C.c_void_p, _SIZE3, C.c_int, C.c_int, C.c_int, C.POINTER(C.c_void_p)]),
    ("clwh_image_wrap", C.c_int, [C.c_void_p, C.c_void_p, _SIZE3, C.c_int, C.c_int, C.POINTER(C.c_void_p)]),
    ("clwh_mem_push", C.c_int, [C.c_void_p, C.c_void_p, C.c_void_p, C.c_size_t]),
    ("clwh_mem_pull", C.c_int, [C.c_void_p, C.c_void_p, C.c_void_p, C.c_size_t]),
    ("clwh_mem_release", C.c_int, [C.c_void_p]),
    ("clwh_host_register", C.c_int, [C.c_void_p, C.c_size_t]),
    ("clwh_host_unregister", C.c_int, [C.c_void_p]),
    ("clwh_mem_device_ptr", C.c_void_p, [C.c_void_p]),
    ("clwh_mem_size", C.c_size_t, [C.c_void_p]),
    ("clwh_mem_mark_dirty", C.c_int, [C.c_void_p]),
    ("clwh_kernel_get", C.c_int, [C.c_void_p, C.c_char_p, C.c_char_p, C.c_char_p, C.POINTER(C.c_void_p)]),
    ("clwh_kernel_release", C.c_int, [C.c_void_p]),
    ("clwh_launch", C.c_int, [C.c_void_p, _SIZE3, _SIZE3, C.POINTER(Arg), C.c_int]),
    ("clwh_render", C.c_int, [C.c_void_p, C.POINTER(RenderDesc)]),
    ("clwh_cache_len", C.c_int64, [C.c_uint32, C.c_uint32, C.c_uint32]),
    ("clwh_accum_len", C.c_int64, [C.c_uint32, C.c_uint32, C.c_int32]),
    ("clwh_accum_resolve", C.c_int, [C.c_void_p, C.c_void_p, C.c_int32, C.c_uint32, C.c_uint32, C.c_void_p,
                                     C.c_void_p, C.POINTER(C.c_float), C.POINTER(C.c_float)]),
    ("clwh_accum_resolve_tiles", C.c_int, [C.c_void_p, C.c_void_p, C.c_int32, C.c_int32, C.c_uint32, C.c_uint32, C.c_void_p,
                                           C.c_void_p, C.POINTER(C.c_float), C.POINTER(C.c_float)]),
    ("clwh_frame_from_tiles", C.c_int, [C.c_void_p, C.c_void_p, C.c_int32, C.c_uint32, C.c_uint32, C.c_void_p]),
    ("clwh_ctx_invalidate_derived", C.c_int, [C.c_void_p, C.c_int]),
    ("clwh_ctx_scene_info", C.c_int, [C.c_void_p, C.POINTER(C.c_uint64), C.POINTER(C.c_uint64), C.POINTER(C.c_int32)]),
    ("clwh_render_projection", C.c_int, [C.c_void_p, C.POINTER(ProjectionDesc)]),
    ("clwh_render_composite", C.c_int, [C.c_void_p, C.POINTER(CompositeDesc)]),
    ("clwh_render_isosurface", C.c_int, [C.c_void_p, C.POINTER(IsosurfaceDesc)]),
    ("clwh_render_slice", C.c_int, [C.c_void_p, C.POINTER(SliceDesc)]),
    ("clwh_mesh_isosurface", C.c_int, [C.c_void_p, C.POINTER(MeshDesc)]),
    ("clwh_segment_grow", C.c_int, [C.c_void_p, C.POINTER(GrowDesc)]),
    ("clwh_volume_apply_mask", C.c_int, [C.c_void_p, C.POINTER(ApplyMaskDesc)]),
    ("clwh_segment_label", C.c_int, [C.c_void_p, C.POINTER(LabelDesc)]),
    ("clwh_labels_to_mask", C.c_int, [C.c_void_p, C.POINTER(LabelsToMaskDesc)]),
    ("clwh_mask_distance", C.c_int, [C.c_void_p, C.POINTER(DistanceDesc)]),
    ("clwh_mask_morph", C.c_int, [C.c_void_p, C.POINTER(MorphDesc)]),
    ("clwh_mask_combine", C.c_int, [C.c_void_p, C.POINTER(MaskCombineDesc)]),
    ("clwh_mask_geodesic", C.c_int, [C.c_void_p, C.POINTER(GeodesicDesc)]),
    ("clwh_geodesic_trace", C.c_int, [C.c_void_p, C.POINTER(GeodesicTraceDesc)]),
    ("clwh_mask_statistics", C.c_int, [C.c_void_p, C.POINTER(MaskStatsDesc)]),
    ("clwh_label_statistics", C.c_int, [C.c_void_p, C.POINTER(LabelStatsDesc)]),
    ("clwh_overlay_slice", C.c_int, [C.c_void_p, C.POINTER(OverlaySliceDesc)]),
    ("clwh_overlay_camera", C.c_int, [C.c_void_p, C.POINTER(OverlayCameraDesc)]),
    ("clwh_sdf_build", C.c_int, [C.c_void_p, C.c_void_p, C.c_char_p, C.c_void_p, C.POINTER(C.c_int32)]),
    ("clwh_buffer_reset", C.c_int, [C.c_void_p, C.c_void_p]),
    ("clwh_cache_exchange_plan", C.c_int, [C.c_void_p, C.c_void_p, C.c_uint64, C.POINTER(C.c_void_p)]),
    ("clwh_cache_apply_contributions", C.c_int, [C.c_void_p, C.c_void_p, C.c_void_p, C.c_void_p, C.c_int32]),
    ("clwh_cache_exchange_plan_release", C.c_int, [C.c_void_p]),
    ("clwh_tf_parse", C.c_int, [C.c_char_p, C.POINTER(Tf)]),
    ("clwh_debug_float_conversions", C.c_int, [C.c_void_p, C.c_void_p, C.c_uint64, C.c_void_p, C.c_void_p]),
    ("clwh_debug_wave_min", C.c_int, [C.c_void_p, C.c_void_p, C.c_uint64, C.c_void_p]),
    ("clwh_debug_device_probe", C.c_int, [C.c_void_p, C.c_int32, C.c_void_p, C.c_uint64, C.c_void_p, C.c_void_p, C.POINTER(C.c_int32)]),
    ("clwh_debug_macro_table", C.c_int, [C.c_void_p, C.c_void_p, C.c_uint64, C.POINTER(C.c_int32)]),
    ("clwh_debug_packed_scene", C.c_int, [C.c_void_p, C.c_int32, C.c_void_p, C.c_uint64, C.POINTER(C.c_int32)]),
    ("clwh_debug_view_data", C.c_int, [C.c_void_p, C.c_int32, C.c_void_p, C.c_uint64, C.POINTER(C.c_int32)]),
    ("clwh_debug_start_table", C.c_int, [C.c_void_p, C.c_void_p, C.c_uint64, C.POINTER(C.c_int32)]),
    ("clwh_debug_start_cert_dmin", C.c_int, [C.c_int32, C.c_int32, C.c_int32, C.POINTER(C.c_float)]),
    ("clwh_debug_hit_records", C.c_int, [C.c_void_p, C.c_void_p, C.c_uint64, C.POINTER(C.c_uint32)]),
    ("clwh_debug_hull_table", C.c_int, [C.c_void_p, C.c_void_p, C.c_uint64, C.POINTER(C.c_int32)]),
    ("clwh_debug_hull_cert_bound", C.c_int, [C.c_int32, C.c_int32, C.c_int32, C.POINTER(C.c_float)]),
    ("clwh_debug_hull_codes", C.c_int, [C.c_void_p, C.c_void_p, C.c_uint64, C.POINTER(C.c_uint32)]),
    ("clwh_debug_hull_planes", C.c_int, [C.c_void_p, C.c_void_p, C.c_uint64, C.POINTER(C.c_uint32)]),
    ("clwh_debug_hull_defer_bound", C.c_int, [C.c_int32, C.c_int32, C.c_int32, C.POINTER(C.c_float)]),
    ("clwh_strerror", C.c_char_p, [C.c_int]),
    ("clwh_last_hip_error", C.c_int, []),
    ("clwh_version", C.c_char_p, []),
    ("clwh_ctx_acquire_from", C.c_int, [C.c_void_p, C.c_void_p]),
    ("clwh_ctx_release_to", C.c_int, [C.c_void_p, C.c_void_p]),
    ("clwh_ctx_set_timing", C.c_int, [C.c_void_p, C.c_int]),
    ("clwh_ctx_timing_read", C.c_int, [C.c_void_p, C.POINTER(C.c_float), C.POINTER(C.c_int32)]),
    ("clwh_ctx_timing_read_all", C.c_int, [C.c_void_p, C.POINTER(C.c_float), C.POINTER(C.c_int32), C.c_int32]),
]
EXPORTED_SYMBOLS = [p[0] for p in _PROTOTYPES]

_lib = None


def lib():
    global _lib
    if _lib is None:
        if not os.path.exists(LIB_PATH):
            raise RuntimeError(
                "libclwhip.so is missing (%s): build it with `python -m cl_volume_renderer_amd.build`; "
                "there is no CPU fallback for the product path" % LIB_PATH)
        L = C.CDLL(LIB_PATH)
        for name, res, args in _PROTOTYPES:
            if not hasattr(L, name) and os.environ.get("CLWH_LIBRARY"):
                continue
            f = getattr(L, name)
            f.restype = res
            f.argtypes = args
        _lib = L
    return _lib


def _check(status, where):
    if status != OK:
        raise ClwhError(status, where)


def parse_tf(source: str) -> Tf:
    tf = Tf()
    _check(lib().clwh_tf_parse(source.encode(), C.byref(tf)), "clwh_tf_parse")
    return tf


def hull_cert_bound(X: int, Y: int, Z: int):
    v = (C.c_float * 2)()
    _check(lib().clwh_debug_hull_cert_bound(X, Y, Z, v), "clwh_debug_hull_cert_bound")
    return float(v[0]), float(v[1])


def hull_defer_bound(X: int, Y: int, Z: int):
    v = (C.c_float * 4)()
    _check(lib().clwh_debug_hull_defer_bound(X, Y, Z, v), "clwh_debug_hull_defer_bound")
    return float(v[0]), int(v[1]), float(v[2]), int(v[3])


def start_cert_dmin(X: int, Y: int, Z: int) -> float:
    v = C.c_float(0)
    _check(lib().clwh_debug_start_cert_dmin(X, Y, Z, C.byref(v)), "clwh_debug_start_cert_dmin")
    return float(v.value)


def cache_len(X, Y, Z) -> int:
    return int(lib().clwh_cache_len(X, Y, Z))


def accum_len(w, h, world=1) -> int:
    return int(lib().clwh_accum_len(w, h, world))


def _handle(mem):
    return mem.h if mem is not None else None


def _fill_overlay(d, frame, source, kind, dims, palette, width, height, n_colours, flags, fill_alpha, outline_alpha, id_range, ids, t_first):
    d.frame = _handle(frame)
    d.region.buffer, d.region.kind = _handle(source), int(kind)
    for k in range(3):
        d.region.dims[k] = int(dims[k])
    d.region.id_lo, d.region.id_hi = int(id_range[0]), int(id_range[1])
    d.paint.palette = _handle(palette)
    d.paint.n_colours = int(n_colours if n_colours is not None else (palette.nbytes // 4 if palette is not None else 0))
    d.paint.flags, d.paint.fill_alpha, d.paint.outline_alpha = int(flags), int(fill_alpha), int(outline_alpha)
    d.paint.ids, d.paint.t_first = _handle(ids), _handle(t_first)
    d.width, d.height = int(width), int(height)


def _fill_view(d, frame, volume, cam_pos, cam_dir, width, height):
    d.frame, d.volume = frame.h, volume.h
    for k in range(3):
        d.cam_pos[k] = float(cam_pos[k])
        d.cam_dir[k] = float(cam_dir[k])
    d.width, d.height = int(width), int(height)


class Mem:
    def __init__(self, ctx, handle, nbytes, dtype=None, shape=None):
        self.ctx, self.h, self.nbytes, self.dtype, self.shape = ctx, C.c_void_p(handle), nbytes, dtype, shape

    def push(self, arr: np.ndarray):
        a = np.ascontiguousarray(arr)
        _check(lib().clwh_mem_push(self.ctx.h, self.h, a.ctypes.data, a.nbytes), "clwh_mem_push")

    def pull(self, dtype=None, shape=None) -> np.ndarray:
        dtype = np.dtype(dtype or self.dtype or np.uint8)
        out = np.empty(self.nbytes // dtype.itemsize, dtype=dtype)
        _check(lib().clwh_mem_pull(self.ctx.h, self.h, out.ctypes.data, out.nbytes), "clwh_mem_pull")
        shape = shape or self.shape
        return out.reshape(shape) if shape else out

    @property
    def device_ptr(self) -> int:
        return int(lib().clwh_mem_device_ptr(self.h) or 0)

    def release(self):
        if self.h:
            _check(lib().clwh_mem_release(self.h), "clwh_mem_release")
            self.h = None


class Kernel:
    def __init__(self, ctx, handle):
        self.ctx, self.h = ctx, C.c_void_p(handle)

    def launch(self, global_size, local_size, *args):
        g = (C.c_size_t * 3)(*(list(global_size) + [0, 0, 0])[:3])
        l = (C.c_size_t * 3)(*(list(local_size) + [0, 0, 0])[:3])
        arr = (Arg * max(len(args), 1))()
        for i, a in enumerate(args):
            if isinstance(a, Mem):
                arr[i].kind, arr[i].v.mem = ARG_MEM, a.h.value
            elif isinstance(a, (float, np.floating)):
                arr[i].kind, arr[i].v.f32 = ARG_F32, float(a)
            elif isinstance(a, np.unsignedinteger):
                arr[i].kind, arr[i].v.u32 = ARG_U32, int(a)
            elif isinstance(a, (int, np.integer)):
                arr[i].kind, arr[i].v.i32 = ARG_I32, int(a)
# ... 538 lines not shown
        finally:
            if table is not None:
                table.release()

    def label_statistics_raw(self, volume: Mem, labels: Mem, stats: Mem, capacity, flags=0):
        d = LabelStatsDesc()
        d.volume, d.labels, d.stats = _handle(volume), _handle(labels), _handle(stats)
        d.capacity, d.flags = int(capacity), int(flags)
        return lib().clwh_label_statistics(self.h, C.byref(d))

    def label_statistics(self, volume: Mem, labels: Mem, capacity, stats: Mem = None) -> Mem:
        own = stats is None
        if own:
            stats = self.buffer(104 * max(int(capacity), 1), REGION_STATS_DTYPE, (max(int(capacity), 1),))
        status = self.label_statistics_raw(volume, labels, stats, capacity)
        if status != OK and own:
            stats.release()
        _check(status, "clwh_label_statistics")
        return stats

    def scene_info(self):
        sid, nb, holders = C.c_uint64(0), C.c_uint64(0), C.c_int32(0)
        _check(lib().clwh_ctx_scene_info(self.h, C.byref(sid), C.byref(nb), C.byref(holders)), "clwh_ctx_scene_info")
        return int(sid.value), int(nb.value), int(holders.value)

    def device_probe(self, which, records: np.ndarray, params=(0, 0, 0, 0), aux: np.ndarray = None) -> np.ndarray:
        w_in, w_out = PROBE_WORDS[which]
        rec = np.ascontiguousarray(records, dtype=np.uint32).reshape(-1, w_in)
        n = rec.shape[0]
        m_in, m_out = self.buffer_from(rec if n else np.zeros(1, np.uint32)), self.buffer(max(n, 1) * w_out * 4, np.uint32)
        m_aux = self.buffer_from(np.ascontiguousarray(aux, dtype=np.uint32)) if aux is not None else None
        try:
            _check(lib().clwh_debug_device_probe(self.h, which, m_in.h, C.c_uint64(n), m_out.h, m_aux.h if m_aux else None,
                                                 (C.c_int32 * 4)(*[int(v) for v in params])), "clwh_debug_device_probe")
            self.finish()
            return m_out.pull().reshape(-1, w_out)[:n]
        finally:
            for m in (m_in, m_out, m_aux):
                if m is not None:
                    m.release()

    def macro_table(self):
        info = (C.c_int32 * 4)()
        _check(lib().clwh_debug_macro_table(self.h, None, C.c_uint64(0), info), "clwh_debug_macro_table")
        out = np.empty((info[2], info[1], info[0], 8), np.uint8)
        _check(lib().clwh_debug_macro_table(self.h, out.ctypes.data_as(C.c_void_p), C.c_uint64(out.nbytes), info), "clwh_debug_macro_table")
        return out, int(info[3])

    def packed_scene(self, which):
        info = (C.c_int32 * 4)()
        _check(lib().clwh_debug_packed_scene(self.h, which, None, C.c_uint64(0), info), "clwh_debug_packed_scene")
        n = info[0] * info[1] * info[2]
        out = (np.empty((n, 512, 2), np.uint32) if which == SCENE_HIT_RECORDS else
               np.empty((n, 512), np.uint8) if which == SCENE_STEP_BYTES else np.empty(n, np.uint32))
        _check(lib().clwh_debug_packed_scene(self.h, which, out.ctypes.data_as(C.c_void_p), C.c_uint64(out.nbytes), info), "clwh_debug_packed_scene")
        return out, (int(info[0]), int(info[1]), int(info[2]))

    def view_data(self, which):
        info = (C.c_int32 * 4)()
        _check(lib().clwh_debug_view_data(self.h, which, None, C.c_uint64(0), info), "clwh_debug_view_data")
        n = info[0] * info[1] * info[2]
        out = np.empty((n, 512), np.int16) if which == VIEW_BRICKS else np.empty(info[3] if which == VIEW_COARSE else n, np.uint32)
        _check(lib().clwh_debug_view_data(self.h, which, out.ctypes.data_as(C.c_void_p), C.c_uint64(out.nbytes), info), "clwh_debug_view_data")
        return out, (int(info[0]), int(info[1]), int(info[2]))

    def start_table(self):
        info = (C.c_int32 * 4)()
        _check(lib().clwh_debug_start_table(self.h, None, C.c_uint64(0), info), "clwh_debug_start_table")
        if not info[3]:
            return None
        out = np.empty((info[2], info[1], info[0]), np.uint8)
        _check(lib().clwh_debug_start_table(self.h, out.ctypes.data_as(C.c_void_p), C.c_uint64(out.nbytes), info), "clwh_debug_start_table")
        return out

    def hull_table(self):
        info = (C.c_int32 * 4)()
        _check(lib().clwh_debug_hull_table(self.h, None, C.c_uint64(0), info), "clwh_debug_hull_table")
        if not info[3]:
            return None
        out = np.empty((info[1], 4), np.float32)
        _check(lib().clwh_debug_hull_table(self.h, out.ctypes.data_as(C.c_void_p), C.c_uint64(out.nbytes), info), "clwh_debug_hull_table")
        return out

    def hull_codes(self):
        n = C.c_uint32(0)
        _check(lib().clwh_debug_hull_codes(self.h, None, C.c_uint64(0), C.byref(n)), "clwh_debug_hull_codes")
        out = np.empty(int(n.value), np.uint32)
        _check(lib().clwh_debug_hull_codes(self.h, out.ctypes.data_as(C.c_void_p), C.c_uint64(out.nbytes), C.byref(n)), "clwh_debug_hull_codes")
        return out[:int(n.value)]

    def hull_planes(self):
        n = C.c_uint32(0)
        _check(lib().clwh_debug_hull_planes(self.h, None, C.c_uint64(0), C.byref(n)), "clwh_debug_hull_planes")
        out = np.empty(int(n.value), np.uint32)
        _check(lib().clwh_debug_hull_planes(self.h, out.ctypes.data_as(C.c_void_p), C.c_uint64(out.nbytes), C.byref(n)), "clwh_debug_hull_planes")
        return out[:int(n.value)]

    def hit_records(self):
        n = C.c_uint32(0)
        _check(lib().clwh_debug_hit_records(self.h, None, C.c_uint64(0), C.byref(n)), "clwh_debug_hit_records")
        out = np.empty((int(n.value), 16), np.uint32)
        _check(lib().clwh_debug_hit_records(self.h, out.ctypes.data_as(C.c_void_p), C.c_uint64(out.nbytes), C.byref(n)), "clwh_debug_hit_records")
        return out[:int(n.value)]

    def image_wrap(self, device_ptr: int, dims, channels, dtype, shape=None) -> Mem:
        dtype = np.dtype(dtype)
        d = (C.c_size_t * 3)(*(list(dims) + [1, 1, 1])[:3])
        h = C.c_void_p()
        _check(lib().clwh_image_wrap(self.h, C.c_void_p(device_ptr), d, channels, _ELEM_OF_DTYPE[dtype], C.byref(h)),
               "clwh_image_wrap")
        n = int(np.prod([max(int(x), 1) for x in list(dims)[:3]])) * channels * dtype.itemsize
        return Mem(self, h.value, n, dtype, shape)

    def acquire_from(self, stream: int):
        _check(lib().clwh_ctx_acquire_from(self.h, C.c_void_p(stream)), "clwh_ctx_acquire_from")

    def release_to(self, stream: int):
        _check(lib().clwh_ctx_release_to(self.h, C.c_void_p(stream)), "clwh_ctx_release_to")

    def finish(self):
        _check(lib().clwh_ctx_finish(self.h), "clwh_ctx_finish")

    def set_timing(self, enabled=True):
        _check(lib().clwh_ctx_set_timing(self.h, 1 if enabled else 0), "clwh_ctx_set_timing")

    def timing_read(self):
        ms, n = C.c_float(0), C.c_int32(0)
        _check(lib().clwh_ctx_timing_read(self.h, C.byref(ms), C.byref(n)), "clwh_ctx_timing_read")
        return float(ms.value), int(n.value)

    def timing_read_all(self):
        n = len(TIMERS)
        ms, cnt = (C.c_float * n)(), (C.c_int32 * n)()
        _check(lib().clwh_ctx_timing_read_all(self.h, ms, cnt, n), "clwh_ctx_timing_read_all")
        return {name: (float(ms[i]), int(cnt[i])) for i, name in enumerate(TIMERS)}

    @property
    def stream(self) -> int:
        return int(lib().clwh_ctx_stream(self.h) or 0)

    def destroy(self):
        if self.h:
            _check(lib().clwh_ctx_destroy(self.h), "clwh_ctx_destroy")
            self.h = None
```

### include/clwh.h

```cpp
#ifndef CLWH_H
#define CLWH_H

#include <stddef.h>
#include <stdint.h>

#ifdef __cplusplus
extern "C" {
#endif

typedef struct clwh_ctx clwh_ctx;
typedef struct clwh_mem clwh_mem;
typedef struct clwh_kernel clwh_kernel;

enum clwh_status {
  CLWH_OK = 0,
  CLWH_ERR_INVALID_VALUE = 1,
  CLWH_ERR_NO_DEVICE = 2,
  CLWH_ERR_OUT_OF_MEMORY = 3,
  CLWH_ERR_HIP = 4,
  CLWH_ERR_UNKNOWN_KERNEL = 5,
  CLWH_ERR_TF_UNSUPPORTED = 6,
  CLWH_ERR_BAD_ARGS = 7,
  CLWH_ERR_BAD_NDRANGE = 8,
  CLWH_ERR_SIZE_MISMATCH = 9,
// ... 383 lines not shown
enum clwh_overlay_flags {
  CLWH_OVERLAY_FILL = 1,
  CLWH_OVERLAY_OUTLINE = 2,
  CLWH_OVERLAY_DENSE = 4
};
typedef struct clwh_overlay_region {
  clwh_mem *buffer;
  int32_t kind;
  uint32_t dims[3];
  uint32_t id_lo, id_hi;
} clwh_overlay_region;
typedef struct clwh_overlay_paint {
  clwh_mem *palette;
  uint32_t n_colours;
  int32_t flags;
  uint32_t fill_alpha, outline_alpha;
  clwh_mem *ids;
  clwh_mem *t_first;
} clwh_overlay_paint;
typedef struct clwh_overlay_slice_desc {
  clwh_mem *frame;
  clwh_overlay_region region;
  clwh_overlay_paint paint;
  float origin[3], du[3], dv[3], normal[3];
  uint32_t width, height;
  int32_t slab_samples;
  float step;
} clwh_overlay_slice_desc;
typedef struct clwh_overlay_camera_desc {
  clwh_mem *frame;
  clwh_overlay_region region;
  clwh_overlay_paint paint;
  float cam_pos[3], cam_dir[3];
  uint32_t width, height;
  float step;
  float t_near, t_far;
  int32_t reserved;
} clwh_overlay_camera_desc;
int clwh_overlay_slice(clwh_ctx *ctx, const clwh_overlay_slice_desc *desc);
int clwh_overlay_camera(clwh_ctx *ctx, const clwh_overlay_camera_desc *desc);

int clwh_sdf_build(clwh_ctx *ctx, clwh_mem *volume, const char *tf_source, clwh_mem *sdf,
                   int32_t *n_launches);

int clwh_buffer_reset(clwh_ctx *ctx, clwh_mem *buffer_volume);

typedef struct clwh_exchange_plan clwh_exchange_plan;
int clwh_cache_exchange_plan(clwh_ctx *ctx, clwh_mem *entries, uint64_t n, clwh_exchange_plan **out);
int clwh_cache_apply_contributions(clwh_ctx *ctx, clwh_exchange_plan *plan, clwh_mem *buffer_volume, clwh_mem *rgb,
                                   int32_t rgb_stride);
int clwh_cache_exchange_plan_release(clwh_exchange_plan *plan);

int clwh_ctx_acquire_from(clwh_ctx *ctx, void *hip_stream);
int clwh_ctx_release_to(clwh_ctx *ctx, void *hip_stream);

#define CLWH_TF_MAX_RULES 16
typedef struct clwh_tf_rule {
  int32_t v_lo, v_hi;
  int32_t g_lo, g_hi;
  int32_t use_gradient;
  int32_t writes_color;
  int32_t terminal;
  int32_t color[4];
} clwh_tf_rule;
typedef struct clwh_tf {
  int32_t n;
  clwh_tf_rule rules[CLWH_TF_MAX_RULES];
} clwh_tf;
int clwh_tf_parse(const char *source, clwh_tf *out);

int clwh_debug_float_conversions(clwh_ctx *ctx, clwh_mem *floats_in, uint64_t n, clwh_mem *i32_out, clwh_mem *u32_out);
int clwh_debug_wave_min(clwh_ctx *ctx, clwh_mem *u32_in, uint64_t n, clwh_mem *u32_out);
enum clwh_probe {
  CLWH_PROBE_ARITH = 0,
  CLWH_PROBE_HASH = 1,
  CLWH_PROBE_HEMISPHERE = 2,
  CLWH_PROBE_RAY = 3,
  CLWH_PROBE_CUT = 4,
  CLWH_PROBE_ENV_EXACT = 5,
  CLWH_PROBE_ENV_FAST = 6,
  CLWH_PROBE_ENV_APPROX = 7,
  CLWH_PROBE_TONE = 8,
  CLWH_PROBE_TAPS = 9,
  CLWH_PROBE_COUNT = 10
};
int clwh_debug_device_probe(clwh_ctx *ctx, int32_t which, clwh_mem *in, uint64_t n, clwh_mem *out, clwh_mem *aux, const int32_t params[4]);
int clwh_debug_macro_table(clwh_ctx *ctx, void *host_out, uint64_t capacity, int32_t info_out[4]);
enum clwh_scene_array { CLWH_SCENE_HIT_RECORDS = 0, CLWH_SCENE_STEP_BYTES = 1, CLWH_SCENE_BRICK_MIN = 2 };
int clwh_debug_packed_scene(clwh_ctx *ctx, int32_t which, void *host_out, uint64_t capacity, int32_t info_out[4]);
enum clwh_view_array { CLWH_VIEW_BRICKS = 0, CLWH_VIEW_TABLE = 1, CLWH_VIEW_DILATED = 2, CLWH_VIEW_COARSE = 3 };
int clwh_debug_view_data(clwh_ctx *ctx, int32_t which, void *host_out, uint64_t capacity, int32_t info_out[4]);
int clwh_debug_start_table(clwh_ctx *ctx, void *host_out, uint64_t capacity, int32_t info_out[4]);
int clwh_debug_start_cert_dmin(int32_t X, int32_t Y, int32_t Z, float *dmin_out);
int clwh_debug_hit_records(clwh_ctx *ctx, void *host_out, uint64_t capacity, uint32_t *n_hits_out);
int clwh_debug_hull_table(clwh_ctx *ctx, void *host_out, uint64_t capacity, int32_t info_out[4]);
int clwh_debug_hull_cert_bound(int32_t X, int32_t Y, int32_t Z, float out[2]);
int clwh_debug_hull_codes(clwh_ctx *ctx, void *host_out, uint64_t capacity, uint32_t *n_hits_out);
int clwh_debug_hull_planes(clwh_ctx *ctx, void *host_out, uint64_t capacity, uint32_t *n_hits_out);
int clwh_debug_hull_defer_bound(int32_t X, int32_t Y, int32_t Z, float out[4]);
const char *clwh_strerror(int status);
int clwh_last_hip_error(void);
const char *clwh_version(void);
int clwh_ctx_set_timing(clwh_ctx *ctx, int enabled);
int clwh_ctx_timing_read(clwh_ctx *ctx, float *total_ms, int32_t *launches);
enum clwh_timer {
  CLWH_TIMER_BOUNCE = 0,
  CLWH_TIMER_PRIMARY = 1,
  CLWH_TIMER_FIXUP = 2,
  CLWH_TIMER_RESOLVE = 3,
  CLWH_TIMER_REPACK = 4,
  CLWH_TIMER_AO = 5,
  CLWH_TIMER_COUNT = 6
};
int clwh_ctx_timing_read_all(clwh_ctx *ctx, float *ms, int32_t *launches, int32_t n);

#ifdef __cplusplus
}
#endif
#endif
```

Before: 46760.

## Add tilted hull-plane certificate to grant or defer early exit for bounce rays

When neither the start nor the hull certificate fires at bounce start, the ray now tries a second hull plane, tilted toward the ray direction and looked up through a separate plane-height array. It either grants an immediate exit or arms a deferred exit within a bounded path length. The deferred-fire threshold and the defer delta are recomputed for a longer step window. Armed lanes that reach the certificate phase early are sent back to marching without a lookup. The aim is to stop more rays from marching all the way out of the volume, at the cost of extra per-ray arithmetic, one more table read and more divergence.

Result: faster. 47820 (median of 6 runs) (+2.3%).

```diff
diff --git a/cl_volume_renderer_amd/csrc/bounce_device.hpp b/cl_volume_renderer_amd/csrc/bounce_device.hpp
--- a/cl_volume_renderer_amd/csrc/bounce_device.hpp
+++ b/cl_volume_renderer_amd/csrc/bounce_device.hpp
@@ -76,6 +76,14 @@
   const float x = z >= 0.0f ? u : copysignf(1.0f - fabsf(v), u), y = z >= 0.0f ? v : copysignf(1.0f - fabsf(u), v);
   const float r = __builtin_amdgcn_rsqf((x * x + y * y) + z * z);
   return f3{x * r, y * r, z * r};
+}
+__device__ __forceinline__ unsigned hull_cell(f3 n) {
+  static_assert(kHullGrid == 64, "cell (i, j) covers u in [i / 32 - 1, (i + 1) / 32 - 1)");
+  const float r = __builtin_amdgcn_rcpf((fabsf(n.x) + fabsf(n.y)) + fabsf(n.z));
+  const float x = n.x * r, y = n.y * r;
+  const float u = n.z >= 0.0f ? x : copysignf(1.0f - fabsf(y), x), v = n.z >= 0.0f ? y : copysignf(1.0f - fabsf(x), y);
+  const int i = (int)fminf(fmaxf(floorf(u * 32.0f + 32.0f), 0.0f), 63.0f), j = (int)fminf(fmaxf(floorf(v * 32.0f + 32.0f), 0.0f), 63.0f);
+  return (unsigned)(j * 64 + i);
 }
 __device__ __forceinline__ bool certify_exit(const RenderArgs &a, f3 p, f3 d, int budget) {
   int away;
@@ -121,6 +129,8 @@
   __device__ void hull_cert(bool, bool, bool) {}
   __device__ void hull_more(bool, bool, bool, bool) {}
   __device__ void hull_fired(bool, bool) {}
+  __device__ void hull_tilt(bool, bool, bool, bool, bool) {}
+  __device__ void hull_late(bool) {}
   __device__ void march_end(uint32_t *, int) {}
   template <bool TWO_RAYS> __device__ void flush(uint32_t *) {}
 };
@@ -177,17 +187,33 @@
     more_tried[1] += (uint32_t)__popcll(__ballot(rebound_tried)); more_granted[1] += (uint32_t)__popcll(__ballot(rebound_granted));
     if (rebound_granted) more_open = 1;
   }
-  __device__ __forceinline__ void hull_fired(bool fired, bool first_leg) {
+  __device__ __forceinline__ void hull_fired(bool fired_any, bool first_leg) {
+    const bool fired = fired_any && !tilt_armed, tilted = fired_any && tilt_armed;
     more_granted[0] += (uint32_t)__popcll(__ballot(fired && first_leg)); more_granted[2] += (uint32_t)__popcll(__ballot(fired && !first_leg));
     if (fired) more_open = first_leg ? 0 : 2;
-  }
+    tilt_granted[1] += (uint32_t)__popcll(__ballot(tilted && first_leg)); tilt_granted[3] += (uint32_t)__popcll(__ballot(tilted && !first_leg));
+    if (tilted) tilt_open = first_leg ? 1 : 3;
+  }
+  uint32_t tilt_tried[4] = {0, 0, 0, 0}, tilt_granted[4] = {0, 0, 0, 0}, tilt_late = 0;
+  int tilt_open = -1;
+  bool tilt_armed = false;
+  __device__ __forceinline__ void hull_tilt(bool tried, bool granted, bool armed, bool starts, bool first_leg) {
+    tilt_tried[0] += (uint32_t)__popcll(__ballot(tried && first_leg)); tilt_tried[2] += (uint32_t)__popcll(__ballot(tried && !first_leg));
+    tilt_granted[0] += (uint32_t)__popcll(__ballot(granted && first_leg)); tilt_granted[2] += (uint32_t)__popcll(__ballot(granted && !first_leg));
+    tilt_tried[1] += (uint32_t)__popcll(__ballot(armed && first_leg)); tilt_tried[3] += (uint32_t)__popcll(__ballot(armed && !first_leg));
+    if (granted) tilt_open = first_leg ? 0 : 2;
+    if (starts) tilt_armed = armed;
+  }
+  __device__ __forceinline__ void hull_late(bool late) { tilt_late += (uint32_t)__popcll(__ballot(late)); }
   __device__ __forceinline__ void march_end(uint32_t *counters, int ev) {
     if (start_open && ev != EV_EXIT) atomicAdd(&counters[CTR_START_WRONG], 1u);
     if (hull_open && ev != EV_EXIT) atomicAdd(&counters[CTR_HULL_WRONG], 1u);
     if (more_open >= 0 && ev != EV_EXIT) atomicAdd(&counters[CTR_HULL_DEFER + 3 * more_open + 2], 1u);
+    if (tilt_open >= 0 && ev != EV_EXIT) atomicAdd(&counters[CTR_HULL_TILT + 3 * tilt_open + 2], 1u);
     start_open = false;
     hull_open = false;
     more_open = -1;
+    tilt_open = -1;
   }
   template <bool TWO_RAYS> __device__ __forceinline__ void flush(uint32_t *counters) {
     atomicAdd(&counters[CTR_STEP_ITERS], step_iters); atomicAdd(&counters[CTR_STEP_LANES], step_lanes);
@@ -200,6 +226,8 @@
     atomicAdd(&counters[CTR_START_TRIED], start_tried); atomicAdd(&counters[CTR_START_GRANTED], start_granted);
     atomicAdd(&counters[CTR_HULL_TRIED], hull_tried); atomicAdd(&counters[CTR_HULL_GRANTED], hull_granted); atomicAdd(&counters[CTR_HULL_BOTH], hull_both);
     for (int k = 0; k < 3; ++k) { atomicAdd(&counters[CTR_HULL_DEFER + 3 * k], more_tried[k]); atomicAdd(&counters[CTR_HULL_DEFER + 3 * k + 1], more_granted[k]); }
+    for (int k = 0; k < 4; ++k) { atomicAdd(&counters[CTR_HULL_TILT + 3 * k], tilt_tried[k]); atomicAdd(&counters[CTR_HULL_TILT + 3 * k + 1], tilt_granted[k]); }
+    atomicAdd(&counters[CTR_HULL_TILT + 12], tilt_late);
   }
 };
 using BounceStats = BounceStatsT<kBounceStats>;
diff --git a/cl_volume_renderer_amd/csrc/clwh_context.hip b/cl_volume_renderer_amd/csrc/clwh_context.hip
--- a/cl_volume_renderer_amd/csrc/clwh_context.hip
+++ b/cl_volume_renderer_amd/csrc/clwh_context.hip
@@ -156,6 +156,7 @@
   if (const char *e = std::getenv("CLWH_TUNE_START_CERT")) t.start_cert = std::atoi(e) != 0;
   if (const char *e = std::getenv("CLWH_TUNE_HULL_CERT")) t.hull_cert = std::atoi(e) != 0;
   if (const char *e = std::getenv("CLWH_TUNE_HULL_DEFER")) t.hull_defer = std::atoi(e) != 0;
+  if (const char *e = std::getenv("CLWH_TUNE_HULL_TILT")) t.hull_tilt = std::atoi(e) != 0;
   return t;
 }
 
diff --git a/cl_volume_renderer_amd/csrc/clwh_host.hpp b/cl_volume_renderer_amd/csrc/clwh_host.hpp
--- a/cl_volume_renderer_amd/csrc/clwh_host.hpp
+++ b/cl_volume_renderer_amd/csrc/clwh_host.hpp
@@ -120,6 +120,7 @@
   int32_t start_cert = 1;
   int32_t hull_cert = 1;
   int32_t hull_defer = 1;
+  int32_t hull_tilt = 1;
   int32_t cert_min_step = -1;
   uint32_t bounce_max_blocks = 2048;
   int32_t sdfbit_waves = 8;
diff --git a/cl_volume_renderer_amd/csrc/clwh_internal.hpp b/cl_volume_renderer_amd/csrc/clwh_internal.hpp
--- a/cl_volume_renderer_amd/csrc/clwh_internal.hpp
+++ b/cl_volume_renderer_amd/csrc/clwh_internal.hpp
@@ -53,6 +53,7 @@
   CTR_STATS_END,
   CTR_QUEUE_STRIDE = 32,
   CTR_HULL_DEFER = CTR_QUEUE_STRIDE * 9, CTR_HULL_DEFER_END = CTR_HULL_DEFER + 9,
+  CTR_HULL_TILT = CTR_HULL_DEFER_END, CTR_HULL_TILT_END = CTR_HULL_TILT + 13,
 };
 struct RenderArgs {
   int32_t X, Y, Z;
@@ -72,6 +73,9 @@
   float hull_delta0;
   uint32_t *hull_planes;
   float hull_defer_delta0;
+  const float *hull_h;
+  float hull_tilt_target;
+  float hull_tilt_gain;
   int32_t NBX, NBY;
   const uint32_t *env;
   int32_t env_w, env_h;
@@ -195,13 +199,13 @@
 constexpr int kHullDeferSteps = 3;
 constexpr float kHullDeferDeficit = 1.5f;
 constexpr int kHullMarginScale = 16;
-inline float hull_defer_delta0(int X, int Y, int Z) {
+inline float hull_defer_delta0(int X, int Y, int Z, int J = kHullDeferSteps) {
   const double longest = (double)(X > Y ? (X > Z ? X : Z) : (Y > Z ? Y : Z));
   const double reach = 1.7320508075688772 * (longest + 1.0), cap = (double)start_cert_cap(X, Y, Z);
   for (int k = 1; k <= 64; ++k) {
     const double delta0 = (double)k / 64.0;
     double t = 0.0;
-    for (int step = 0; step < 70 - 5 - kHullDeferSteps && t <= reach; ++step) {
+    for (int step = 0; step < 70 - 5 - J && t <= reach; ++step) {
       const double m = (double)(long long)(t * delta0 / 1.7320508075688772) - 2.0;
       const double bound = m > cap ? cap : m;
       t += bound < 1.0 ? 1.0 : bound;
@@ -210,7 +214,10 @@
   }
   return 2.0f;
 }
-hipError_t launch_hull_table(const int2 *ends, const uint32_t *regular, float4 *hull, int X, int Y, int Z, hipStream_t s);
+constexpr int kHullTiltSteps = 16;
+constexpr float kHullTiltMargin = 0.0625f;
+constexpr int kHullTiltPath = 48;
+hipError_t launch_hull_table(const int2 *ends, const uint32_t *regular, float4 *hull, float *hull_h, int X, int Y, int Z, hipStream_t s);
 constexpr uint64_t kStartTableBudget = 2ull << 30;
 hipError_t launch_primary(const RenderArgs &a, hipStream_t s);
 hipError_t launch_bounce(const RenderArgs &a, hipStream_t s);
diff --git a/cl_volume_renderer_amd/csrc/clwh_render.hip b/cl_volume_renderer_amd/csrc/clwh_render.hip
--- a/cl_volume_renderer_amd/csrc/clwh_render.hip
+++ b/cl_volume_renderer_amd/csrc/clwh_render.hip
@@ -1,4 +1,5 @@
 #include <algorithm>
+#include <cmath>
 #include <cstdio>
 #include <cstring>
 #include <mutex>
@@ -19,7 +20,7 @@
 
 struct PackedLayout {
   int X, Y, Z, NBX, NBY, NBZ, mshift, MNX, MNY, MNZ;
-  size_t records, n_bricks, off_stepb, off_brick_min, off_macro, off_start, off_hull_ends, off_hull, bytes;
+  size_t records, n_bricks, off_stepb, off_brick_min, off_macro, off_start, off_hull_ends, off_hull, off_hull_h, bytes;
   bool start_table;
   bool hull_table;
 };
@@ -31,6 +32,12 @@
   return t.hull_cert != 0 && wants_start_table(t, tf, volume) && volume->dims[0] <= (size_t)kHullMaxDim && volume->dims[1] <= (size_t)kHullMaxDim &&
          volume->dims[2] <= (size_t)kHullMaxDim;
 }
+static void hull_tilt_target(float delta, float &target, float &gain) {
+  const double t = std::min((double)delta + (double)kHullTiltMargin, 0.984375);
+  target = (float)t;
+  gain = (float)(t / std::sqrt(1.0 - t * t));
+}
+
 static PackedLayout packed_layout(const clwh_mem *volume, int forced_macro_shift, bool start_table, bool hull_table) {
   PackedLayout L;
   L.X = (int)volume->dims[0]; L.Y = (int)volume->dims[1]; L.Z = (int)volume->dims[2];
@@ -49,7 +56,8 @@
   L.hull_table = hull_table;
   L.off_hull = L.off_hull_ends + (hull_table ? (size_t)L.Y * L.Z * sizeof(int2) : 0u);
   L.off_hull = (L.off_hull + 15u) & ~(size_t)15u;
-  L.bytes = hull_table ? L.off_hull + (size_t)kHullPlanes * sizeof(float4) : L.off_start + (start_table ? 16u + (size_t)L.X * L.Y * L.Z : 0u);
+  L.off_hull_h = L.off_hull + (size_t)kHullPlanes * sizeof(float4);
+  L.bytes = hull_table ? L.off_hull_h + (size_t)kHullPlanes * sizeof(float) : L.off_start + (start_table ? 16u + (size_t)L.X * L.Y * L.Z : 0u);
   return L;
 }
 
@@ -116,7 +124,7 @@
       int2 *ends = L.hull_table ? reinterpret_cast<int2 *>(data + L.off_hull_ends) : nullptr;
       const hipError_t e = launch_start_table(r.stepb, data + L.off_start + 16u, reinterpret_cast<uint32_t *>(data + L.off_start), ends, L.X, L.Y, L.Z, L.NBX, L.NBY, L.NBZ, ctx->stream);
       if (e != hipSuccess || !L.hull_table) return e;
-      return launch_hull_table(ends, reinterpret_cast<const uint32_t *>(data + L.off_start), reinterpret_cast<float4 *>(data + L.off_hull), L.X, L.Y, L.Z, ctx->stream);
+      return launch_hull_table(ends, reinterpret_cast<const uint32_t *>(data + L.off_start), reinterpret_cast<float4 *>(data + L.off_hull), reinterpret_cast<float *>(data + L.off_hull_h), L.X, L.Y, L.Z, ctx->stream);
     }));
   HIP_TRY(hipEventRecord(entry->ready.ev, ctx->stream));
   ctx->scene = entry;
@@ -257,6 +265,11 @@
   a.macro = packed + L.off_macro;
   a.start_free = L.start_table ? packed + L.off_start + 16u : nullptr;
   a.hull = L.hull_table ? reinterpret_cast<const float4 *>(packed + L.off_hull) : nullptr;
+  a.hull_h = L.hull_table && ctx->tune.hull_defer != 0 && ctx->tune.hull_tilt != 0 ? reinterpret_cast<const float *>(packed + L.off_hull_h) : nullptr;
+  if (a.hull_h) {
+    a.hull_defer_delta0 = hull_defer_delta0(a.X, a.Y, a.Z, kHullTiltSteps);
+    hull_tilt_target(a.hull_defer_delta0, a.hull_tilt_target, a.hull_tilt_gain);
+  }
   a.macro_shift = L.mshift;
   a.MNX = L.MNX; a.MNY = L.MNY; a.MNZ = L.MNZ;
   bool zero_may_hit = a.tf.border_class != 0;
@@ -385,7 +398,7 @@
 
 #ifdef CLVR_BOUNCE_STATS
 static int print_bounce_stats(clwh_ctx *ctx, const RenderArgs &a) {
-  uint32_t h[CTR_HULL_DEFER_END];
+  uint32_t h[CTR_HULL_TILT_END];
   HIP_TRY(hipMemcpyAsync(h, a.counters, sizeof h, hipMemcpyDeviceToHost, ctx->stream));
   HIP_TRY(hipStreamSynchronize(ctx->stream));
   auto per = [&](int sum, int n) { return h[n] ? (double)h[sum] / h[n] : 0.0; };
@@ -404,8 +417,12 @@
                (double)a.hull_delta0);
   const uint32_t *m = h + CTR_HULL_DEFER;
   std::fprintf(stderr, "[bounce stats] hull certificates tried/granted/wrong: first legs deferred=%u/%u/%u rebounds at once=%u/%u/%u rebounds deferred=%u/%u/%u; "
-               "J=%d D=%.4g defer_delta0=%.6f; look-ups=%u\n", m[0], m[1], m[2], m[3], m[4], m[5], m[6], m[7], m[8], kHullDeferSteps, (double)kHullDeferDeficit,
-               (double)a.hull_defer_delta0, h[CTR_CERT_LANES] - ((CLVR_BOUNCE_STATS + 0) == 2 ? m[1] + m[7] : 0u));
+               "J=%d D=%.4g defer_delta0=%.6f; look-ups=%u\n", m[0], m[1], m[2], m[3], m[4], m[5], m[6], m[7], m[8], a.hull_h ? kHullTiltSteps : kHullDeferSteps, (double)kHullDeferDeficit,
+               (double)a.hull_defer_delta0, h[CTR_CERT_LANES] - ((CLVR_BOUNCE_STATS + 0) == 2 ? m[1] + m[7] + h[CTR_HULL_TILT + 4] + h[CTR_HULL_TILT + 10] : 0u) - h[CTR_HULL_TILT + 12]);
+  const uint32_t *t = h + CTR_HULL_TILT;
+  std::fprintf(stderr, "[bounce stats] tilted planes (%s) tried/granted/wrong: first legs at once=%u/%u/%u first legs deferred=%u/%u/%u rebounds at once=%u/%u/%u "
+               "rebounds deferred=%u/%u/%u; armed lanes that got there late and were sent back without a look-up=%u; target=%.6f\n", a.hull_h ? "on" : "off", t[0], t[1], t[2], t[3], t[4], t[5],
+               t[6], t[7], t[8], t[9], t[10], t[11], t[12], (double)a.hull_tilt_target);
   return CLWH_OK;
 }
 #endif
@@ -670,6 +687,30 @@
   return CLWH_OK;
 }
 
+int clwh_debug_hull_tilt_bound(int32_t X, int32_t Y, int32_t Z, float out[6]) {
+  if (!out || X < 1 || Y < 1 || Z < 1) return CLWH_ERR_INVALID_VALUE;
+  out[0] = hull_defer_delta0(X, Y, Z, kHullTiltSteps);
+  out[1] = (float)kHullTiltSteps;
+  out[2] = (float)kHullTiltPath;
+  out[3] = kHullTiltMargin;
+  hull_tilt_target(out[0], out[4], out[5]);
+  return CLWH_OK;
+}
+
+int clwh_debug_hull_h(clwh_ctx *ctx, void *host_out, uint64_t capacity, int32_t info_out[4]) {
+  if (!ctx || !info_out) return CLWH_ERR_INVALID_VALUE;
+  if (!ctx->scene) return CLWH_ERR_BAD_ARGS;
+  const PackedLayout L = scene_layout(ctx);
+  info_out[0] = kHullGrid; info_out[1] = kHullPlanes; info_out[2] = 0; info_out[3] = L.hull_table ? 1 : 0;
+  if (!host_out || !L.hull_table) return CLWH_OK;
+  const size_t bytes = (size_t)kHullPlanes * sizeof(float);
+  if (capacity < bytes || ctx->scene->data.bytes != L.bytes) return CLWH_ERR_SIZE_MISMATCH;
+  HIP_TRY(hipSetDevice(ctx->device));
+  HIP_TRY(hipMemcpyAsync(host_out, ctx->scene->data.as<uint8_t>() + L.off_hull_h, bytes, hipMemcpyDeviceToHost, ctx->stream));
+  HIP_TRY(hipStreamSynchronize(ctx->stream));
+  return CLWH_OK;
+}
+
 int clwh_debug_hull_planes(clwh_ctx *ctx, void *host_out, uint64_t capacity, uint32_t *n_hits_out) {
   if (!ctx || !n_hits_out) return CLWH_ERR_INVALID_VALUE;
   PrimaryHits &p = ctx->primary;
diff --git a/cl_volume_renderer_amd/csrc/probe_kernels.hip b/cl_volume_renderer_amd/csrc/probe_kernels.hip
--- a/cl_volume_renderer_amd/csrc/probe_kernels.hip
+++ b/cl_volume_renderer_amd/csrc/probe_kernels.hip
@@ -1,4 +1,4 @@
-#include "render_device.hpp"
+#include "bounce_device.hpp"
 
 namespace clvr {
 
@@ -14,6 +14,7 @@
     case CLWH_PROBE_ENV_APPROX: return {3u, 2u};
     case CLWH_PROBE_TONE: return {4u, 1u};
     case CLWH_PROBE_TAPS: return {3u, 3u};
+    case CLWH_PROBE_HULL: return {5u, 5u};
     default: return {0u, 0u};
   }
 }
@@ -93,6 +94,14 @@
       o[2] = (uint32_t)((uint64_t)e >> 32);
       break;
     }
+    case CLWH_PROBE_HULL: {
+      const f3 n = hull_direction(r[0]);
+      const float scale = __uint_as_float(r[1]);
+      put_f3(o, n);
+      o[3] = hull_cell(f3{n.x * scale, n.y * scale, n.z * scale});
+      o[4] = hull_cell(f3_at(r + 2));
+      break;
+    }
     default: break;
   }
 }
diff --git a/cl_volume_renderer_amd/csrc/render_kernels.hip b/cl_volume_renderer_amd/csrc/render_kernels.hip
--- a/cl_volume_renderer_amd/csrc/render_kernels.hip
+++ b/cl_volume_renderer_amd/csrc/render_kernels.hip
@@ -55,6 +55,8 @@
   const bool hull_defer = hull_cert && a.hull_planes != nullptr;
   const int entry_hi_bits = hull_defer ? 3 : 8;
   const uint32_t *hull_words = hull_defer ? a.hull_planes : a.hull_codes;
+  const bool hull_tilt = hull_defer && a.hull_h != nullptr;
+  constexpr uint32_t kFireDefer = (uint32_t)(70 - kHullDeferSteps) * kOneStep, kFireTilt = (uint32_t)(70 - kHullTiltSteps) * kOneStep;
   bool exhausted = false;
   BounceStats stats;
 
@@ -97,13 +99,18 @@
         const int n_cert = __popcll(__ballot(st == ST_CERT));
         if (n_cert != 0 && (n_cert >= cert_min_lanes || __popcll(__ballot(st == ST_MARCH)) < a.step_min_lanes)) {
           stats.cert_begin(st, n_cert);
-          const bool fired = !USE_GRAD && st == ST_CERT && (march & kArmed) != 0u && (march & ~kArmed) >= (uint32_t)(70 - kHullDeferSteps) * kOneStep;
+          const bool was_armed = !USE_GRAD && st == ST_CERT && (march & kArmed) != 0u;
+          const bool fired = was_armed && (march & ~kArmed) >= (hull_tilt ? kFireTilt : kFireDefer);
+          const bool late = hull_tilt && was_armed && !fired && sd < cert_at;
           stats.hull_fired(fired, i == 8);
+          stats.hull_late(late);
           if (st == ST_CERT) {
             if (!USE_GRAD) march &= ~kArmed;
             int away;
             if (fired && !kStartCertVerify) {
               st = ST_EVENT + EV_EXIT;
+            } else if (late) {
+              st = ST_MARCH;
             } else if (certify_exit(a, ray.origin, ray.direction, (int)(march >> 24), away)) {
               st = ST_EVENT + EV_EXIT;
             } else {
@@ -288,6 +295,8 @@
     bool hc_tried = false, hc_granted = false;
     bool rb_tried = false, rb_granted = false;
     uint32_t armed_path = 0u;
+    bool tl_tried = false, tl_granted = false, tl_armed = false;
+    bool started = false;
     if (st >= ST_EVENT) {
       const int ev = st - ST_EVENT;
       bool start_path = (ev == EV_START);
@@ -357,22 +366,39 @@
           else { hc_tried = tried && m >= 0.0f; hc_granted = granted; }
           if (tried && dir_ok && !sc_granted && m < 0.0f && m >= -kHullDeferDeficit && dn >= a.hull_defer_delta0)
             armed_path = (uint32_t)ceilf(-m * __builtin_amdgcn_rcpf(dn) * (1.0f + 0x1p-19f));
+          if (hull_tilt && dir_ok && !granted && !sc_granted && armed_path == 0u) {
+            const f3 n0{tried ? n.x : bn.x, tried ? n.y : bn.y, tried ? n.z : bn.z};
+            const float c = dot3(dir, n0);
+            const float lambda = c >= a.hull_tilt_target ? 0.0f : a.hull_tilt_gain * __builtin_amdgcn_sqrtf(fmaxf(1.0f - c * c, 0.0f)) - c;
+            const unsigned k2 = hull_cell(f3{n0.x + lambda * dir.x, n0.y + lambda * dir.y, n0.z + lambda * dir.z});
+            const f3 n2 = hull_direction(k2);
+            const float dn2 = dot3(dir, n2), m2 = dot3(n2, nr.origin) - a.hull_h[k2];
+            tl_tried = true;
+            if (m2 >= 0.0f && dn2 >= a.hull_delta0) {
+              tl_granted = true;
+            } else if (m2 < 0.0f && dn2 >= a.hull_defer_delta0) {
+              const float need = ceilf(-m2 * __builtin_amdgcn_rcpf(dn2) * (1.0f + 0x1p-19f));
+              if (need <= (float)kHullTiltPath) { armed_path = (uint32_t)need; tl_armed = true; }
+            }
+          }
         }
         ray = nr;
       }
 
-      if ((sc_granted || hc_granted || rb_granted) && !kStartCertVerify) {
+      if ((sc_granted || hc_granted || rb_granted || tl_granted) && !kStartCertVerify) {
         st = ST_EVENT + EV_EXIT;
       } else {
         sd = (int)(vol.template step_i<SMALL>(f2i(ray.origin.x), f2i(ray.origin.y), f2i(ray.origin.z)) & 0x7Fu);
         march = 70u * kOneStep + kCertReady;
         if (armed_path != 0u) march = kArmed + 70u * kOneStep + kCertReady - armed_path;
         st = ST_MARCH;
+        started = true;
       }
     }
     stats.start_cert(sc_tried, sc_granted);
     stats.hull_cert(hc_tried, hc_granted, hc_granted && sc_granted);
-    stats.hull_more(rb_tried, rb_granted, armed_path != 0u && st == ST_MARCH, i == 8);
+    stats.hull_more(rb_tried, rb_granted, armed_path != 0u && !tl_armed && st == ST_MARCH, i == 8);
+    stats.hull_tilt(tl_tried, tl_granted, tl_armed && st == ST_MARCH, started, i == 8);
   }
 #undef COLD_ENTRY_HI
 #undef COLD
diff --git a/cl_volume_renderer_amd/csrc/scene_kernels.hip b/cl_volume_renderer_amd/csrc/scene_kernels.hip
--- a/cl_volume_renderer_amd/csrc/scene_kernels.hip
+++ b/cl_volume_renderer_amd/csrc/scene_kernels.hip
@@ -315,7 +315,7 @@
   }
   if (best > -INFINITY) atomicMax(&best_out[4u * k + 3u], ordered_bits(best));
 }
-__global__ __launch_bounds__(256) void k_hull_finish(const uint32_t *__restrict__ regular, float4 *__restrict__ hull) {
+__global__ __launch_bounds__(256) void k_hull_finish(const uint32_t *__restrict__ regular, float4 *__restrict__ hull, float *__restrict__ hull_h) {
   const unsigned k = blockIdx.x * 256u + threadIdx.x;
   const f3 n = hull_direction(k);
   const uint32_t o = reinterpret_cast<const uint32_t *>(hull)[4u * k + 3u];
@@ -323,15 +323,16 @@
   float h = INFINITY;
   if (o != 0u && *regular != 0u) h = (__uint_as_float(b) + ((fmaxf(n.x, 0.0f) + fmaxf(n.y, 0.0f)) + fmaxf(n.z, 0.0f))) + kHullSlack;
   hull[k] = make_float4(n.x, n.y, n.z, h);
-}
-hipError_t launch_hull_table(const int2 *ends, const uint32_t *regular, float4 *hull, int X, int Y, int Z, hipStream_t s) {
+  hull_h[k] = h;
+}
+hipError_t launch_hull_table(const int2 *ends, const uint32_t *regular, float4 *hull, float *hull_h, int X, int Y, int Z, hipStream_t s) {
   (void)X;
   const hipError_t e = hipMemsetAsync(hull, 0, (size_t)kHullPlanes * sizeof(float4), s);
   if (e != hipSuccess) return e;
   const int n_rows = Y * Z;
   hipLaunchKernelGGL(k_hull_support, dim3((unsigned)kHullPlanes / 256u, ((unsigned)n_rows + (unsigned)kHullRows - 1u) / (unsigned)kHullRows), dim3(256), 0, s, ends, Y, n_rows,
                      reinterpret_cast<uint32_t *>(hull));
-  hipLaunchKernelGGL(k_hull_finish, dim3((unsigned)kHullPlanes / 256u), dim3(256), 0, s, regular, hull);
+  hipLaunchKernelGGL(k_hull_finish, dim3((unsigned)kHullPlanes / 256u), dim3(256), 0, s, regular, hull, hull_h);
   return hipGetLastError();
 }
 
diff --git a/cl_volume_renderer_amd/ffi.py b/cl_volume_renderer_amd/ffi.py
--- a/cl_volume_renderer_amd/ffi.py
+++ b/cl_volume_renderer_amd/ffi.py
@@ -34,8 +34,8 @@
 OVERLAY_FILL, OVERLAY_OUTLINE, OVERLAY_DENSE = 1, 2, 4
 SHADE_LIGHT, SHADE_AO = 0, 1
 (PROBE_ARITH, PROBE_HASH, PROBE_HEMISPHERE, PROBE_RAY, PROBE_CUT, PROBE_ENV_EXACT, PROBE_ENV_FAST, PROBE_ENV_APPROX, PROBE_TONE,
- PROBE_TAPS) = range(10)
-PROBE_WORDS = ((6, 12), (1, 1), (7, 6), (10, 3), (6, 4), (3, 1), (3, 2), (3, 2), (4, 1), (3, 3))
+ PROBE_TAPS, PROBE_HULL) = range(11)
+PROBE_WORDS = ((6, 12), (1, 1), (7, 6), (10, 3), (6, 4), (3, 1), (3, 2), (3, 2), (4, 1), (3, 3), (5, 5))
 SCENE_HIT_RECORDS, SCENE_STEP_BYTES, SCENE_BRICK_MIN = range(3)
 VIEW_BRICKS, VIEW_TABLE, VIEW_DILATED, VIEW_COARSE = range(4)
 TIMERS = ("bounce", "primary", "fixup", "resolve", "repack", "ao")
@@ -400,6 +400,8 @@
     ("clwh_debug_hull_codes", C.c_int, [C.c_void_p, C.c_void_p, C.c_uint64, C.POINTER(C.c_uint32)]),
     ("clwh_debug_hull_planes", C.c_int, [C.c_void_p, C.c_void_p, C.c_uint64, C.POINTER(C.c_uint32)]),
     ("clwh_debug_hull_defer_bound", C.c_int, [C.c_int32, C.c_int32, C.c_int32, C.POINTER(C.c_float)]),
+    ("clwh_debug_hull_tilt_bound", C.c_int, [C.c_int32, C.c_int32, C.c_int32, C.POINTER(C.c_float)]),
+    ("clwh_debug_hull_h", C.c_int, [C.c_void_p, C.c_void_p, C.c_uint64, C.POINTER(C.c_int32)]),
     ("clwh_strerror", C.c_char_p, [C.c_int]),
     ("clwh_last_hip_error", C.c_int, []),
     ("clwh_version", C.c_char_p, []),
@@ -453,6 +455,12 @@
     v = (C.c_float * 4)()
     _check(lib().clwh_debug_hull_defer_bound(X, Y, Z, v), "clwh_debug_hull_defer_bound")
     return float(v[0]), int(v[1]), float(v[2]), int(v[3])
+
+
+def hull_tilt_bound(X: int, Y: int, Z: int):
+    v = (C.c_float * 6)()
+    _check(lib().clwh_debug_hull_tilt_bound(X, Y, Z, v), "clwh_debug_hull_tilt_bound")
+    return float(v[0]), int(v[1]), int(v[2]), float(v[3]), float(v[4]), float(v[5])
 
 
 def start_cert_dmin(X: int, Y: int, Z: int) -> float:
@@ -1157,6 +1165,15 @@
         _check(lib().clwh_debug_hull_table(self.h, out.ctypes.data_as(C.c_void_p), C.c_uint64(out.nbytes), info), "clwh_debug_hull_table")
         return out
 
+    def hull_h(self):
+        info = (C.c_int32 * 4)()
+        _check(lib().clwh_debug_hull_h(self.h, None, C.c_uint64(0), info), "clwh_debug_hull_h")
+        if not info[3]:
+            return None
+        out = np.empty(info[1], np.float32)
+        _check(lib().clwh_debug_hull_h(self.h, out.ctypes.data_as(C.c_void_p), C.c_uint64(out.nbytes), info), "clwh_debug_hull_h")
+        return out
+
     def hull_codes(self):
         n = C.c_uint32(0)
         _check(lib().clwh_debug_hull_codes(self.h, None, C.c_uint64(0), C.byref(n)), "clwh_debug_hull_codes")
diff --git a/include/clwh.h b/include/clwh.h
--- a/include/clwh.h
+++ b/include/clwh.h
@@ -489,7 +489,8 @@
   CLWH_PROBE_ENV_APPROX = 7,
   CLWH_PROBE_TONE = 8,
   CLWH_PROBE_TAPS = 9,
-  CLWH_PROBE_COUNT = 10
+  CLWH_PROBE_HULL = 10,
+  CLWH_PROBE_COUNT = 11
 };
 int clwh_debug_device_probe(clwh_ctx *ctx, int32_t which, clwh_mem *in, uint64_t n, clwh_mem *out, clwh_mem *aux, const int32_t params[4]);
 int clwh_debug_macro_table(clwh_ctx *ctx, void *host_out, uint64_t capacity, int32_t info_out[4]);
@@ -505,6 +506,8 @@
 int clwh_debug_hull_codes(clwh_ctx *ctx, void *host_out, uint64_t capacity, uint32_t *n_hits_out);
 int clwh_debug_hull_planes(clwh_ctx *ctx, void *host_out, uint64_t capacity, uint32_t *n_hits_out);
 int clwh_debug_hull_defer_bound(int32_t X, int32_t Y, int32_t Z, float out[4]);
+int clwh_debug_hull_tilt_bound(int32_t X, int32_t Y, int32_t Z, float out[6]);
+int clwh_debug_hull_h(clwh_ctx *ctx, void *host_out, uint64_t capacity, int32_t info_out[4]);
 const char *clwh_strerror(int status);
 int clwh_last_hip_error(void);
 const char *clwh_version(void);
```
